# SidRama/Longitudinal-VAE

Hardware: AMD Instinct MI355X
Metric: ELBO-steps/sec (exact-KL L-VAE step, Health-MNIST N=4096 L=16) (higher is better)
Workload: dtype f16x3-split (fp32-equivalent)

## Files before the change

### include/lvae_hip.h

```cpp
#ifndef LVAE_HIP_H
#define LVAE_HIP_H

#include <stddef.h>
#include <stdint.h>

#ifdef __cplusplus
extern "C" {
#endif

#define LVAE_MAX_COMP 16
#define LVAE_MAX_FAC 4
#define LVAE_ERR_LAUNCH (-1000)

enum lvae_factor_kind {
  LVAE_CAT = 0,
  LVAE_BIN = 1,
  LVAE_RBF = 2,
  LVAE_PER = 3,
  LVAE_LIN = 4
};

typedef struct lvae_kernel_spec {
  int32_t n_comp;
  int32_t n_params;
  int32_t n_fac[LVAE_MAX_COMP];
  int32_t scale_idx[LVAE_MAX_COMP];
  int32_t kind[LVAE_MAX_COMP][LVAE_MAX_FAC];
  int32_t dim[LVAE_MAX_COMP][LVAE_MAX_FAC];
  int32_t param_idx[LVAE_MAX_COMP][LVAE_MAX_FAC];
} lvae_kernel_spec;

typedef struct lvae_xview {
  const double* ptr;
  int64_t stride_b;
  int64_t stride_l;
  int64_t ld;
} lvae_xview;


int lvae_gram_f64(const lvae_kernel_spec* spec, lvae_xview x1, lvae_xview x2, int nb, int L, int n1,
                  int n2, const double* params, const double* diag, double* out, int64_t ostride_b,
                  int64_t ostride_l, int64_t ldo, void* stream);
int lvae_gram_f32(const lvae_kernel_spec* spec, lvae_xview x1, lvae_xview x2, int nb, int L, int n1,
                  int n2, const double* params, const double* diag, float* out, int64_t ostride_b,
                  int64_t ostride_l, int64_t ldo, void* stream);

size_t lvae_gram_bwd_workspace_size(int nb, int L, int n1, int n2);
int lvae_gram_bwd_f64(const lvae_kernel_spec* spec, lvae_xview x1, lvae_xview x2, int nb, int L, int n1,
                      int n2, const double* params, const double* G, int64_t gstride_b,
                      int64_t gstride_l, int64_t ldg, double* dparams, double* ddiag, void* workspace,
                      void* stream);

size_t lvae_gram_bwd_x2_workspace_size(int nb, int L, int n1, int n2, int Q);
int lvae_gram_bwd_x2_f64(const lvae_kernel_spec* spec, lvae_xview x1, lvae_xview x2, int nb, int L, int n1, int n2,
                         int Q, const double* params, const double* G, int64_t gstride_b, int64_t gstride_l,
                         int64_t gstride_i, int64_t gstride_j, double* dx2, void* workspace, void* stream);

size_t lvae_gram_matvec_workspace_size(int n1, int n2, int L);
int lvae_gram_matvec_f64(const lvae_kernel_spec* spec, const double* x1, int64_t ld1, int n1, const double* x2,
                         int64_t ld2, int n2, int L, const double* params, const double* diag, const double* v,
                         int64_t ld_v, double* out, int64_t ld_out, void* workspace, void* stream);

int lvae_kl_closed_padded_n(int n);
size_t lvae_kl_closed_workspace_size(int n, int L);


int lvae_kl_closed_fwd_f32(const lvae_kernel_spec* spec, const double* x, int ldx, int n, int L,
                           const double* params, const double* noise, const double* mu, const double* logv,
                           int ld_mu, double* kl, int32_t* info, void* workspace, int need_bwd,
                           void* stream);
int lvae_kl_closed_factor_f32(const lvae_kernel_spec* spec, const double* x, int ldx, int n, int L,
                              const double* params, const double* noise, int32_t* info, void* workspace,
                              void* stream);
int lvae_kl_closed_reduce_f32(const lvae_kernel_spec* spec, const double* x, int ldx, int n, int L,
                              const double* params, const double* noise, const double* mu, const double* logv,
                              int ld_mu, double* kl, void* workspace, int need_bwd, void* stream);

int lvae_kl_closed_bwd_f32(const lvae_kernel_spec* spec, const double* x, int ldx, int n, int L,
                           const double* params, const double* mu, const double* logv, int ld_mu,
                           const double* gkl, double* dmu, double* dlogv, double* dparams, double* dnoise,
                           void* workspace, void* stream);
int lvae_kl_closed_bwd_latent_f32(int n, int L, const double* logv, int ld_mu, const double* gkl, double* dmu,
                                  double* dlogv, void* workspace, void* stream);
int lvae_kl_closed_bwd_hyper_f32(const lvae_kernel_spec* spec, const double* x, int ldx, int n, int L,
                                 const double* params, const double* gkl, double* dparams, double* dnoise,
                                 void* workspace, void* stream);

int lvae_kl_closed_refine_state(int n, int L, const void* workspace, double* est, int32_t* flag, void* stream);

int lvae_kl_closed_hyper_state(int n, int L, const void* workspace, int32_t* on, void* stream);

int lvae_kl_closed_resid_state(int n, int L, const void* workspace, int32_t* covflag, int32_t* binned,
                               void* stream);

size_t lvae_spd_inv_chol_scratch_size(int np_, int L);
int lvae_spd_inv_chol_f32(int np_, int L, float* A, void* scratch, float* Ainv, double* logdet, int32_t* info,
                          void* stream);

int lvae_potrf_f64(int n, int L, const double* A, int64_t lda, int64_t stride_a, double* Lout, int64_t ldo,
                   int64_t stride_o, double* logdet, int32_t* info, void* stream);
size_t lvae_potrf_f32_workspace_size(int n, int L);
int lvae_potrf_f32(int n, int L, const float* A, int64_t lda, int64_t stride_a, float* Lout, int64_t ldo,
                   int64_t stride_o, double* logdet, int32_t* info, void* workspace, void* stream);
size_t lvae_trsm_workspace_size(int n, int L);
int lvae_trsm_f64(int trans, int n, int nrhs, int L, const double* Lf, int64_t ldl, int64_t stride_l, double* B,
                  int64_t ldb, int64_t stride_b, void* workspace, void* stream);
int lvae_trsm_f32(int trans, int n, int nrhs, int L, const float* Lf, int64_t ldl, int64_t stride_l, float* B,
                  int64_t ldb, int64_t stride_b, void* workspace, void* stream);
int lvae_potrs_f64(int n, int nrhs, int L, const double* Lf, int64_t ldl, int64_t stride_l, double* B, int64_t ldb,
                   int64_t stride_b, void* workspace, void* stream);
int lvae_potrs_f32(int n, int nrhs, int L, const float* Lf, int64_t ldl, int64_t stride_l, float* B, int64_t ldb,
                   int64_t stride_b, void* workspace, void* stream);


int lvae_spd_inv_small_f64(int n, int batch, const double* A, int64_t stride, double* Ainv,
                           int64_t stride_out, double* logdet, int32_t* info, void* stream);

int lvae_gemm_small_f64(int ta, int tb, int m, int n, int k, double alpha, const double* A, int lda,
                        int64_t sa1, int64_t sa2, const double* B, int ldb, int64_t sb1, int64_t sb2,
                        double beta, double* C, int ldc, int64_t sc1, int64_t sc2, int nb1, int nb2,
                        void* stream);

typedef struct lvae_hensman_dims {
  int32_t L, M, P_b, T, Q;
  double P_tot;
  double eps;
  int32_t natural_gradient;
  double ng_prior_share;
  const int32_t* seg_len;
  double n_total;
} lvae_hensman_dims;

size_t lvae_hensman_workspace_size(const lvae_hensman_dims* d);
size_t lvae_hensman_iH_offset(const lvae_hensman_dims* d);

int lvae_hensman_fwd_f64(const lvae_kernel_spec* spec0, const lvae_kernel_spec* spec1,
                         const lvae_hensman_dims* d, const double* x, const double* z, const double* m,
                         const double* H, const double* mu, const double* logv, const double* params0,
                         const double* params1, const double* noise, double* kld, double* grad_m,
                         double* grad_H, int32_t* info, void* workspace, void* stream);
int lvae_hensman_fwd_part_f64(int part, const lvae_kernel_spec* spec0, const lvae_kernel_spec* spec1,
                              const lvae_hensman_dims* d, const double* x, const double* z, const double* m,
                              const double* H, const double* mu, const double* logv, const double* params0,
                              const double* params1, const double* noise, double* kld, double* grad_m,
                              double* grad_H, int32_t* info, void* workspace, void* stream);

int lvae_hensman_bwd_f64(const lvae_kernel_spec* spec0, const lvae_kernel_spec* spec1,
                         const lvae_hensman_dims* d, const double* x, const double* z, const double* m,
                         const double* H, const double* mu, const double* logv, const double* params0,
                         const double* params1, const double* noise, const double* gkld, double* dmu,
                         double* dlogv, double* dparams0, double* dparams1, double* dnoise, double* dm,
                         double* dH, void* workspace, void* stream);

size_t lvae_natgrad_workspace_size(int L, int M);
int lvae_natgrad_update_f64(int L, int M, double* m, double* H, const double* grad_m,
                            const double* grad_H, double lr, const double* iH, int32_t* info,
                            void* workspace, void* stream);

typedef struct lvae_dubo_dims {
  int32_t L, M, P, T, Q;
  double eps;
} lvae_dubo_dims;

size_t lvae_dubo_workspace_size(const lvae_dubo_dims* d);

int lvae_dubo_fwd_f64(const lvae_kernel_spec* spec0, const lvae_kernel_spec* spec1, const lvae_dubo_dims* d,
                      const double* x, const double* z, const double* mu, const double* logv,
                      const double* params0, const double* params1, const double* noise, double* dubo,
                      int32_t* info, void* workspace, void* stream);
int lvae_dubo_bwd_f64(const lvae_kernel_spec* spec0, const lvae_kernel_spec* spec1, const lvae_dubo_dims* d,
                      const double* x, const double* z, const double* mu, const double* logv,
                      const double* params0, const double* params1, const double* noise, const double* gdubo,
                      double* dmu, double* dlogv, double* dparams0, double* dparams1, double* dnoise,
                      void* workspace, void* stream);

typedef struct lvae_gp_elbo_dims {
  int32_t L, M, P, T, Q, S;
  double eps;
} lvae_gp_elbo_dims;

size_t lvae_gp_elbo_workspace_size(const lvae_gp_elbo_dims* d);

int lvae_gp_elbo_fwd_f64(const lvae_kernel_spec* spec0, const lvae_kernel_spec* spec1, const lvae_gp_elbo_dims* d,
                         const double* x, const double* z, const double* y, const double* params0,
                         const double* params1, const double* noise, double* elbo, int32_t* info,
                         void* workspace, void* stream);
int lvae_gp_elbo_bwd_f64(const lvae_kernel_spec* spec0, const lvae_kernel_spec* spec1, const lvae_gp_elbo_dims* d,
                         const double* x, const double* z, const double* y, const double* params0,
                         const double* params1, const double* noise, const double* gelbo, double* dy,
                         double* dparams0, double* dparams1, double* dnoise, void* workspace, void* stream);

int lvae_dubo_fwd_seg_f64(const lvae_kernel_spec* spec0, const lvae_kernel_spec* spec1, const lvae_dubo_dims* d,
                          const int32_t* seg_len, const double* x, const double* z, const double* mu,
                          const double* logv, const double* params0, const double* params1, const double* noise,
                          double* dubo, int32_t* info, void* workspace, void* stream);
int lvae_dubo_bwd_seg_f64(const lvae_kernel_spec* spec0, const lvae_kernel_spec* spec1, const lvae_dubo_dims* d,
                          const int32_t* seg_len, const double* x, const double* z, const double* mu,
                          const double* logv, const double* params0, const double* params1, const double* noise,
                          const double* gdubo, double* dmu, double* dlogv, double* dparams0, double* dparams1,
                          double* dnoise, void* workspace, void* stream);
int lvae_gp_elbo_fwd_seg_f64(const lvae_kernel_spec* spec0, const lvae_kernel_spec* spec1,
                             const lvae_gp_elbo_dims* d, const int32_t* seg_len, const double* x, const double* z,
                             const double* y, const double* params0, const double* params1, const double* noise,
                             double* elbo, int32_t* info, void* workspace, void* stream);
int lvae_gp_elbo_bwd_seg_f64(const lvae_kernel_spec* spec0, const lvae_kernel_spec* spec1,
                             const lvae_gp_elbo_dims* d, const int32_t* seg_len, const double* x, const double* z,
                             const double* y, const double* params0, const double* params1, const double* noise,
                             const double* gelbo, double* dy, double* dparams0, double* dparams1, double* dnoise,
                             void* workspace, void* stream);

size_t lvae_bound_dz_workspace_size(int L, int M, int N, int Q);
int lvae_dubo_bwd_z_f64(const lvae_kernel_spec* spec0, const lvae_dubo_dims* d, const double* x, const double* z,
                        const double* params0, double* dz, void* workspace, void* zworkspace, void* stream);
int lvae_gp_elbo_bwd_z_f64(const lvae_kernel_spec* spec0, const lvae_gp_elbo_dims* d, const double* x,
                           const double* z, const double* params0, double* dz, void* workspace, void* zworkspace,
                           void* stream);
int lvae_hensman_bwd_z_f64(const lvae_kernel_spec* spec0, const lvae_hensman_dims* d, const double* x,
                           const double* z, const double* params0, double* dz, void* workspace, void* zworkspace,
                           void* stream);

int lvae_relu_maxpool2_fwd_f32(const float* x, int64_t planes, int H, int W, float* y, uint8_t* idx,
                               void* stream);
int lvae_relu_maxpool2_bwd_f32(const float* gy, const float* y, const uint8_t* idx, int64_t planes, int H,
                               int W, float* gx, void* stream);
size_t lvae_relu_maxpool2_bias_workspace_size(int N, int C);
int lvae_relu_maxpool2_bias_fwd_f32(const float* x, const float* bias, int N, int C, int H, int W, float* y,
                                    uint8_t* idx, void* stream);
int lvae_relu_maxpool2_bias_bwd_f32(const float* gy, const float* y, const uint8_t* idx, int N, int C, int H, int W,
                                    float* gx, float* db, void* workspace, void* stream);
int lvae_conv1_relu_maxpool2_fwd_f32(const float* x, const float* w, const float* bias, int N, int C, int H, int W,
                                     float* y, uint8_t* idx, void* stream);
int lvae_conv3x3_relu_maxpool2_fwd_f32(const float* x, const float* w, const float* bias, int N, int Cin, int C, int H,
                                       int W, float* y, uint8_t* idx, void* stream);
size_t lvae_conv3x3_pool_wgrad_workspace_size(int N, int C, int Cin);
int lvae_conv3x3_pool_wgrad_f32(const float* gy, const float* y, const uint8_t* idx, const float* x, int N, int C,
                                int Cin, int H, int W, float* dw, float* db, void* workspace, void* stream);
size_t lvae_conv3x3_pool_dgrad_lds(int C, int H, int W);
int lvae_conv3x3_pool_dgrad_f32(const float* gy, const float* y, const uint8_t* idx, const float* w, int N, int C,
                                int Cin, int H, int W, float* gx, void* stream);
size_t lvae_deconv2_sigmoid_workspace_size(int N, int Cin, int Hi, int Wi);
int lvae_deconv2_sigmoid_fwd_f32(const float* z, const float* w, const float* bias, int N, int Cin, int Hi, int Wi,
                                 float* out, void* stream);
int lvae_deconv2_sigmoid_bwd_f32(const float* g, const float* out, const float* z, const float* w, int N, int Cin,
                                 int Hi, int Wi, float* gz, float* dw, float* db, void* workspace, void* stream);
int lvae_deconv4s2_relu_fwd_f32(const float* x, const float* w, const float* bias, int N, int Cin, int Cout, int Hi,
                                int Wi, float* y, void* stream);
size_t lvae_deconv4s2_relu_bwd_workspace_size(int N, int Cin, int Cout);
int lvae_deconv4s2_relu_bwd_f32(const float* gy, const float* y, const float* x, const float* w, int N, int Cin,
                                int Cout, int Hi, int Wi, float* dx, float* dw, float* db, void* workspace,
                                void* stream);

size_t lvae_predict_workspace_size(int L, int M, int P, int T, int Nt);
int lvae_predict_f64(const lvae_kernel_spec* spec0, const lvae_kernel_spec* spec1, int L, int M, int Q, int P,
                     int T, const int32_t* seg_len, const int32_t* include, const double* x,
                     const double* mu, const double* z, int Nt, const double* test_x,
                     const double* params0, const double* params1, const double* noise, double eps,
                     double* out, int32_t* info, void* workspace, void* stream);

size_t lvae_predict_exact_workspace_size(int n, int nt, int L);
int lvae_predict_exact_f64(const lvae_kernel_spec* spec, const double* x, int64_t ldx, int n, int L,
                           const double* params, const double* noise, const double* mu, int64_t ld_mu,
                           const double* tx, int64_t ldt, int nt, double* out, int64_t ld_out, int32_t* info,
                           void* workspace, void* stream);

size_t lvae_predict_exact_var_workspace_size(int n, int nt, int L, int chunk);
int lvae_predict_exact_var_f64(const lvae_kernel_spec* spec, const double* x, int64_t ldx, int n, int L,
                               const double* params, const double* noise, const double* mu, int64_t ld_mu,
                               const double* tx, int64_t ldt, int nt, double* out_mean, int64_t ld_out,
                               double* out_var, int64_t ld_var, int add_noise, int chunk, int32_t* info,
                               void* workspace, void* stream);

size_t lvae_predict_var_workspace_size(int L, int M, int P, int T, int Nt);
int lvae_predict_var_f64(const lvae_kernel_spec* spec0, const lvae_kernel_spec* spec1, int L, int M, int Q, int P,
                         int T, const int32_t* seg_len, const int32_t* include, const double* x, const double* mu,
                         const double* z, int Nt, const double* test_x, int n_groups, const int32_t* group_subject,
                         const int32_t* group_start, const double* params0, const double* params1,
                         const double* noise, double eps, double* out, double* out_var, int add_noise, int32_t* info,
                         void* workspace, void* stream);

int lvae_set_early_stream(void* stream);

enum lvae_phase {
  LVAE_PH_GRAM = 0, LVAE_PH_POTRF = 1 , LVAE_PH_POTRI = 2 , LVAE_PH_KL_REDUCE = 3, LVAE_PH_SYRK = 4,
  LVAE_PH_GRAM_BWD = 5, LVAE_PH_BWD_ELEM = 6, LVAE_PH_HENSMAN_FWD = 7, LVAE_PH_HENSMAN_BWD = 8,
  LVAE_PH_NATGRAD = 9, LVAE_PH_SWEEP_UPD = 10 ,
  LVAE_PH_HB_SLAB = 11 , LVAE_N_PHASES = 12
};
int lvae_prof_enable(int on);
int lvae_prof_collect(double* ms, int32_t* count, int n_phases);

const char* lvae_version(void);

int lvae_vae_loss_fwd_f32(const float* recon, const float* x, const float* mask, const float* log_vy, int B, int d,
                          float* mse, float* nll, float* msum, void* stream);
size_t lvae_vae_loss_bwd_partials(int B);
int lvae_vae_loss_bwd_f32(const float* recon, const float* x, const float* mask, const float* log_vy, const float* msum,
                          const float* g_mse, int64_t g_mse_stride, const float* g_nll, int64_t g_nll_stride, int B,
                          int d, float* d_recon, float* dlv_part, void* stream);
int lvae_reparam_fwd_f32(const float* mu, const float* log_var, const float* eps, int64_t n, float* z, void* stream);
int lvae_reparam_bwd_f32(const float* gz, const float* log_var, const float* eps, int64_t n, float* g_log_var,
                         void* stream);
int lvae_param_pack_fwd_f64(int n_raw, int L, int P, const int* cols, const double* const* raws,
                            const double* const* mlogs, double* out, void* stream);
int lvae_bias_relu_fwd_f32(float* y, const float* bias, int N, int C, int HW, void* stream);
size_t lvae_act_bwd_workspace_size(int N, int C);
int lvae_act_bwd_f32(const float* gy, const float* y, int N, int C, int HW, int relu, float* g, float* db,
                     void* workspace, void* stream);
int lvae_step_terms_fwd(const float* mse, const float* nll, int B, const double* kld, float c, double ks, double w,
                        int use_nll, float* rec, float* nl, double* net, double* kd, void* stream);
int lvae_step_terms_bwd(const double* g_net, const float* g_rec, const float* g_nl, const double* g_kd, float c,
                        double ks, double w, int use_nll, float* g_mse, float* g_nll, double* g_kld, void* stream);
int lvae_param_pack_bwd_f64(int n_raw, int L, int P, const int* cols, const double* const* raws,
                            const double* const* mlogs, const double* g, int64_t g_stride0, int64_t g_stride1,
                            double* grad, void* stream);

#ifdef __cplusplus
}
#endif
#endif
```

### longitudinal-vae_amd/csrc/chol_inv.hip

```cpp
#include "prof.hpp"
#include "pv_lds.hpp"
#include "side_stream.hpp"
#include "x3_c16.hpp"

#ifndef LVAE_CI_C16
#define LVAE_CI_C16 1
#endif
#ifndef LVAE_PV_BTRI
#define LVAE_PV_BTRI 1
#endif
#ifndef LVAE_PV_SAMEAB
#define LVAE_PV_SAMEAB 1
#endif
#ifndef LVAE_CI_KREV
#define LVAE_CI_KREV 1
#endif

namespace lvae {

constexpr bool kCiC16 = LVAE_CI_C16 != 0;

#ifndef LVAE_CI_PIPE_MAX_L
#define LVAE_CI_PIPE_MAX_L 2
#endif
// ... 1397 lines not shown
      const int64_t oc = c16_off(l, np_, i * kSwB, j * kSwB);
      c16_tile_planes_out(acc, [&](int) { return -inv * sy; }, g.oh + oc, g.ol + oc);
    } else {
      ci_planes_out(acc, -inv, sy, g.oh + ot, g.ol + ot, np_);
    }
    ci_transposed_out(acc, -inv, lds, [&](int c, int r0, f32x4 v) {
      const int64_t o = kCiC16 ? c16_off(l, np_, j * kSwB + c, i * kSwB + r0) : ott + (int64_t)c * np_ + r0;
      ci_split4(v, sy, g.oth + o, g.otl + o);
    });
    if (threadIdx.x == 0) S.ysc[sl + (int64_t)i * nt + j] = sy;
  } else {
    if constexpr (MODE == kCiLauumKL) {
#pragma unroll
      for (int a = 0; a < 4; ++a)
#pragma unroll
        for (int b = 0; b < 2; ++b) acc[a][b] *= inv;
    }
    const float osc = MODE == kCiLauumKL ? 1.f : inv;
    float* O = g.Kinv + l * np2 + (int64_t)i * kSwB * np_ + (int64_t)j * kSwB;
    float* Ot = g.Kinv + l * np2 + (int64_t)j * kSwB * np_ + (int64_t)i * kSwB;
    const __amdgpu_buffer_rsrc_t ro = __builtin_amdgcn_make_buffer_rsrc(O, (short)0, 0x7fffffff, 0x00020000);
    const int lane = threadIdx.x & 63, w = threadIdx.x >> 6;
    const int vo = (((w >> 2) * 128 + 4 * (lane >> 5)) * np_ + (w & 3) * 64 + (lane & 31)) * 4;
    if (!g.pre) {
#pragma unroll
      for (int a = 0; a < 4; ++a)
#pragma unroll
        for (int e = 0; e < 16; ++e)
#pragma unroll
          for (int b = 0; b < 2; ++b)
            __builtin_amdgcn_raw_buffer_store_b32(__float_as_uint(acc[a][b][e] * osc), ro, vo,
                                                  ((32 * a + (e & 3) + 8 * (e >> 2)) * np_ + 32 * b) * 4, 0);
    }
    if constexpr (MODE == kCiLauumKL) {
      ci_kl_partials(acc, 1.f, g, l, i, j, kl_mu, kl_part);
      const int64_t tb = l * np2 + (int64_t)i * kSwB * np_ + (int64_t)j * kSwB;
      const int64_t tbt = l * np2 + (int64_t)j * kSwB * np_ + (int64_t)i * kSwB;
      const bool hbm = g.bh_out && g.hbon && *g.hbon;
      _Float16* const bho = hbm ? nullptr : g.bh_out;
      _Float16* const blo = hbm ? nullptr : g.bl_out;
      const float sb = bho ? g.bsc[l] : 0.f;
      if (bho && kCiBC16) {
        const int64_t tc = c16_off(l, np_, i * kSwB, j * kSwB);
        c16_tile_planes_out(acc, [&](int b) { return sb * kl_sv[kSwB + sx_col(b)]; }, bho + tc, blo + tc);
      } else if (bho) {
        const __amdgpu_buffer_rsrc_t rh = __builtin_amdgcn_make_buffer_rsrc(bho + tb, (short)0, 0x7fffffff, 0x00020000);
        const __amdgpu_buffer_rsrc_t rl = __builtin_amdgcn_make_buffer_rsrc(blo + tb, (short)0, 0x7fffffff, 0x00020000);
        const int lane = threadIdx.x & 63, w = threadIdx.x >> 6;
        const int vb = (((w >> 2) * 128 + 4 * (lane >> 5)) * np_ + (w & 3) * 64 + (lane & 31)) * 2;
#pragma unroll
        for (int b = 0; b < 2; ++b) {
          const float mc = sb * kl_sv[kSwB + sx_col(b)];
#pragma unroll
          for (int a = 0; a < 4; ++a)
#pragma unroll
            for (int e = 0; e < 16; ++e) {
              const float y = acc[a][b][e] * mc;
              const _Float16 yh = (_Float16)y;
              const _Float16 yl = (_Float16)(y - (float)yh);
              const int so = ((32 * a + (e & 3) + 8 * (e >> 2)) * np_ + 32 * b) * 2;
              __builtin_amdgcn_raw_buffer_store_b16(__builtin_bit_cast(unsigned short, yh), rh, vb, so, 0);
              __builtin_amdgcn_raw_buffer_store_b16(__builtin_bit_cast(unsigned short, yl), rl, vb, so, 0);
            }
        }
      }
      if (i != j && (bho || hbm || LVAE_KL_MIRROR))
        ci_transposed_out(acc, 1.f, lds, [&](int c, int r0, f32x4 v) {
          if (hbm || LVAE_KL_MIRROR) *reinterpret_cast<f32x4*>(Ot + (int64_t)c * np_ + r0) = v;
          if (bho) {
            const f32x4 s4 = *reinterpret_cast<const f32x4*>(&kl_sv[r0]);
            const int64_t o = kCiBC16 ? c16_off(l, np_, j * kSwB + c, i * kSwB + r0) : tbt + (int64_t)c * np_ + r0;
            ci_split4(v * s4, sb, bho + o, blo + o);
          }
        });
    } else if (i != j) {
      ci_transposed_out(acc, inv, lds, [&](int c, int r0, f32x4 v) {
        *reinterpret_cast<f32x4*>(Ot + (int64_t)c * np_ + r0) = v;
      });
    }
  }
}


#define CI_GEMM_LDS                                                                     \
  __shared__ __attribute__((aligned(16))) _Float16 lds[2 * 4 * kSxPart];                \
  __shared__ float sprod[64];                                                           \
  __shared__ uint32_t red;                                                              \
  __shared__ float kl_mu[2 * kSwB], kl_sv[2 * kSwB], kl_part[6 * kSwB];

template <int MODE>
__global__ __launch_bounds__(512) void ci_gemm_kernel(CiGemmArgs g, CiScratch S) {
  CI_GEMM_LDS
  ci_gemm_body<MODE>(g, S, blockIdx.x + g.bid0, lds, sprod, &red, kl_mu, kl_sv, kl_part);
}

template <int M1, int M2>
__global__ __launch_bounds__(512) void ci_pair_kernel(CiGemmArgs g1, CiGemmArgs g2, CiScratch S, int n1) {
  CI_GEMM_LDS
  if ((int)blockIdx.x < n1)
    ci_gemm_body<M1>(g1, S, blockIdx.x, lds, sprod, &red, kl_mu, kl_sv, kl_part);
  else
    ci_gemm_body<M2>(g2, S, blockIdx.x - n1, lds, sprod, &red, kl_mu, kl_sv, kl_part);
}

size_t ci_scratch_bytes(int np_, int L) { return CiScratch(nullptr, np_, L).bytes; }
int ci_factor_f32(int np_, int L, float* A, void* scratch, _Float16* YT, float* Kinv, double* logdet,
                  int32_t* info, hipStream_t st, float* lout = nullptr);

int ci_factor_f32(int np_, int L, float* A, void* scratch, _Float16* YT, float* Kinv, double* logdet,
                  int32_t* info, hipStream_t st, float* lout) {
  if (np_ <= 0 || np_ % kSwB || np_ / kSwB > 64) return -1;
  if (L <= 0) return -2;
  CiScratch S((char*)scratch, np_, L);
  S.lout = lout;
  const int nt = S.nt;
  const int64_t full = (int64_t)L * np_ * np_;
  _Float16* YTh = YT;
  _Float16* YTl = YT + full;
  _Float16* XTh = reinterpret_cast<_Float16*>(Kinv);
  _Float16* XTl = XTh + full;
  _Float16* Yh = XTh;
  _Float16* Yl = XTl;
  auto ok = [](hipError_t e) { return e == hipSuccess; };
  bool pipe = false;
  static const bool early_env = !getenv("LVAE_CI_TRTRI_EARLY") || atoi(getenv("LVAE_CI_TRTRI_EARLY")) != 0;
  static const int free_env = getenv("LVAE_CI_EARLY_FREE") ? atoi(getenv("LVAE_CI_EARLY_FREE")) : -1;
  bool early = false;
  int s_top = 1, ecap = 0;
  while (2 * s_top < nt) s_top *= 2;
  SideStream* sd = nullptr;
  auto trtri_level = [&](int h, int i0, int ni, bool do_x, bool do_y, hipStream_t q, int cap) {
    const int per = ni * h * h, nwg = per * L;
    if (nwg <= 0) return;
    if (do_x) {
      CiGemmArgs gx{S.Lh, S.Ll, YTh, YTl, nullptr, nullptr, XTh, XTl, nullptr, np_, nt, h, per, nwg, i0};
      for (int b0 = 0; b0 < nwg; b0 += cap > 0 ? cap : nwg) {
        gx.bid0 = b0;
        ci_gemm_kernel<kCiX><<<min(nwg - b0, cap > 0 ? cap : nwg), 512, 0, q>>>(gx, S);
      }
    }
    if (do_y) {
      CiGemmArgs gy{Yh, Yl, XTh, XTl, Yh, Yl, YTh, YTl, nullptr, np_, nt, h, per, nwg, i0};
      for (int b0 = 0; b0 < nwg; b0 += cap > 0 ? cap : nwg) {
        gy.bid0 = b0;
        ci_gemm_kernel<kCiY><<<min(nwg - b0, cap > 0 ? cap : nwg), 512, 0, q>>>(gy, S);
      }
    }
  };
  {
    ProfScope ps(LVAE_PH_POTRF, st);
    std::lock_guard<std::recursive_mutex> lock(side_mutex());
    LVAE_TRY(side_stream(sd));
    (void)zero_async(logdet, sizeof(double) * L, st);
    (void)zero_async(info, sizeof(int32_t) * L, st);
    (void)zero_async(S.cnt, CiScratch::cnt_bytes(L, nt), st);
    if (!ok(hipEventRecord(sd->fork, st)) || !ok(hipStreamWaitEvent(sd->s, sd->fork, 0))) return LVAE_ERR_LAUNCH;
    const bool fuse = L <= kCiFuseMaxL;
    const int pmode = lout ? 0 : ci_pipe_mode(np_, L);
    static const bool split_env = !getenv("LVAE_PIVOT_SPLIT") || atoi(getenv("LVAE_PIVOT_SPLIT")) != 0;
    const bool split = split_env;
    static const bool pair = getenv("LVAE_CI_PAIR") && atoi(getenv("LVAE_CI_PAIR")) != 0;
    static const bool la = getenv("LVAE_CI_LOOKAHEAD") && atoi(getenv("LVAE_CI_LOOKAHEAD")) != 0;
    const bool u128 = getenv("LVAE_CI_U128") && atoi(getenv("LVAE_CI_U128")) != 0;
    const bool uring = getenv("LVAE_CI_URING") && atoi(getenv("LVAE_CI_URING")) != 0;
    pipe = pmode > 0;
    hipStreamCaptureStatus cap_st = hipStreamCaptureStatusNone;
    if (!ok(hipStreamIsCapturing(st, &cap_st))) return LVAE_ERR_LAUNCH;
    early = early_env && fuse && !pipe && !lout && nt >= 2 && sd->early && sd->early != st &&
            cap_st == hipStreamCaptureStatusNone;
    {
      const int pvwg = split ? kCiPvG * ((L + 7) / 8 * 8) : L;
      ecap = max(sd->cus - (free_env >= 0 ? free_env : pvwg), max(sd->cus / 4, 1));
    }
    if (fuse) {
      ci_pivot_kernel<1><<<L, 1024, 0, sd->s>>>(A, np_, 0, S, logdet, info, 0, L, g_pivot_prof);
      if (!ok(hipEventRecord(sd->piv[0], sd->s))) return LVAE_ERR_LAUNCH;
      if (nt > 1) ci_prep0_kernel<<<dim3(nt - 1, L), 256, 0, st>>>(A, np_, S);
      if (!ok(hipEventRecord(sd->c, st))) return LVAE_ERR_LAUNCH;
      for (int m = 0; m < nt; ++m) {
        if (m + 1 < nt) {
          if (!ok(hipStreamWaitEvent(sd->s, m == 0 ? sd->c : sd->u2p[(m - 1) & 1], 0))) return LVAE_ERR_LAUNCH;
          if (split) {
            const int Lr = (L + 7) / 8 * 8;
            ci_pivot_kernel<kCiPvG><<<kCiPvG * Lr, 1024, 0, sd->s>>>(A, np_, m + 1, S, logdet, info, 1, L, g_pivot_prof);
          } else {
            ci_pivot_kernel<1><<<L, 1024, 0, sd->s>>>(A, np_, m + 1, S, logdet, info, 1, L, g_pivot_prof);
          }
          if (!ok(hipEventRecord(sd->piv[(m + 1) & 1], sd->s))) return LVAE_ERR_LAUNCH;
        }
        if (!ok(hipStreamWaitEvent(st, sd->piv[m & 1], 0))) return LVAE_ERR_LAUNCH;
        if (pipe && pair) {
          ProfScope pt(LVAE_PH_POTRI, st);
          const int npn = nt - m - 1, ny = m + 16;
          CiGemmArgs gp{nullptr, nullptr, nullptr, nullptr, nullptr, nullptr, nullptr, nullptr, nullptr, np_, nt, m,
                        max(npn, 1), npn * L, 0};
          CiGemmArgs gy{nullptr, nullptr, nullptr, nullptr, nullptr, nullptr, YTh, YTl, nullptr, np_, nt, m, ny, ny * L, 0};
          ci_pair_kernel<kCiPanel, kCiTrY><<<(npn + ny) * L, 512, 0, st>>>(gp, gy, S, npn * L);
          const int n1 = max(nt - m - 2, 0), n2 = max(nt - m - 2, 0) * max(nt - m - 1, 0) / 2, nu = n1 + n2;
          const int perx = (nt - m - 1) * (m + 1), perl = pmode == 2 ? (m + 1) * (m + 2) / 2 : 0;
          CiGemmArgs gu{nullptr, nullptr, nullptr, nullptr, nullptr, nullptr, nullptr, nullptr, A, np_, nt, m,
                        max(nu, 1), nu * L, n1};
          CiGemmArgs gx{S.Lh, S.Ll, YTh, YTl, nullptr, nullptr, nullptr, nullptr, Kinv, np_, nt, m, max(perx + perl, 1),
                        (perx + perl) * L, perx};
          if (nu + perx + perl > 0) ci_pair_kernel<kCiU12c, kCiTrX><<<(nu + perx + perl) * L, 512, 0, st>>>(gu, gx, S, nu * L);
          if (m + 1 < nt && !ok(hipEventRecord(sd->u2p[m & 1], st))) return LVAE_ERR_LAUNCH;
          continue;
        }
        if (m + 1 < nt) {
          ci_panel_kernel<<<dim3(nt - m - 1, L), 512, 0, st>>>(S, np_, m);
          if (early && m == s_top - 1) {
            if (!ok(hipEventRecord(sd->efork, st)) || !ok(hipStreamWaitEvent(sd->early, sd->efork, 0)))
              return LVAE_ERR_LAUNCH;
            {
              ProfScope pe(LVAE_PH_POTRI, sd->early);
              ci_diag_copy_kernel<<<dim3(16 * s_top, L), 256, 0, sd->early>>>(S, np_, Yh, Yl, YTh, YTl, 0);
              for (int h = 1; h < s_top; h *= 2) trtri_level(h, 0, s_top / (2 * h), true, true, sd->early, ecap);
              trtri_level(s_top, 0, 1, true, false, sd->early, ecap);
            }
            if (!ok(hipEventRecord(sd->edone, sd->early))) return LVAE_ERR_LAUNCH;
          }
          const int n1 = nt - m - 2, n2 = (nt - m - 2) * (nt - m - 1) / 2;
          if (n2 > 0 && la && n2 > 1) {
            ProfScope pu(LVAE_PH_SWEEP_UPD, st);
            ci_update_kernel<kCiU12><<<(n1 + 1) * L, 512, 0, st>>>(A, S, np_, m, 1, L, n1, 0);
            if (!ok(hipEventRecord(sd->u2p[m & 1], st))) return LVAE_ERR_LAUNCH;
            ci_update_kernel<kCiU12><<<(n2 - 1) * L, 512, 0, st>>>(A, S, np_, m, n2 - 1, (n2 - 1) * L, 0, 1);
          } else {
            if (n2 > 0) {
              ProfScope pu(LVAE_PH_SWEEP_UPD, st);
              if (u128) {
                ci_update128_kernel<<<4 * (n1 + n2) * L, 256, 0, st>>>(A, S, np_, m, n2, 4 * (n1 + n2) * L, n1);
                ci_prep0_kernel<<<dim3(n1, L), 256, 0, st>>>(A, np_, S, m + 1);
              } else if (uring) {
                ci_update_ring_kernel<kCiU12><<<(n1 + n2) * L, 512, 0, st>>>(A, S, np_, m, n2, n2 * L, n1);
              } else {
                ci_update_kernel<kCiU12><<<(n1 + n2) * L, 512, 0, st>>>(A, S, np_, m, n2, n2 * L, n1);
              }
            }
            if (!ok(hipEventRecord(sd->u2p[m & 1], st))) return LVAE_ERR_LAUNCH;
          }
        }
        if (pipe) {
          ProfScope pt(LVAE_PH_POTRI, st);
          const int pery = m + 16;
          CiGemmArgs gy{nullptr, nullptr, nullptr, nullptr, nullptr, nullptr, YTh, YTl, nullptr, np_, nt, m, pery,
                        pery * L, 0};
          ci_gemm_kernel<kCiTrY><<<pery * L, 512, 0, st>>>(gy, S);
          const int perx = (nt - m - 1) * (m + 1), perl = pmode == 2 ? (m + 1) * (m + 2) / 2 : 0;
          if (perx + perl > 0) {
            CiGemmArgs gx{S.Lh, S.Ll, YTh, YTl, nullptr, nullptr, nullptr, nullptr, Kinv, np_, nt, m, perx + perl,
                          (perx + perl) * L, perx};
            ci_gemm_kernel<kCiTrX><<<(perx + perl) * L, 512, 0, st>>>(gx, S);
          }
        }
      }
    } else {
      if (nt > 1) ci_prep0_kernel<<<dim3(nt - 1, L), 256, 0, sd->s>>>(A, np_, S);
      ci_pivot_kernel<1><<<L, 1024, 0, sd->s>>>(A, np_, 0, S, logdet, info, 0, L, g_pivot_prof);
      if (nt > 1) ci_panel_kernel<<<dim3(nt - 1, L), 512, 0, sd->s>>>(S, np_, 0);
      if (!ok(hipEventRecord(sd->prep, sd->s))) return LVAE_ERR_LAUNCH;
      for (int k = 0; k + 1 < nt; ++k) {
        if (!ok(hipStreamWaitEvent(st, sd->prep, 0))) return LVAE_ERR_LAUNCH;
        const int n1 = nt - k - 1;
        ci_update_kernel<kCiU1><<<n1 * L, 512, 0, st>>>(A, S, np_, k, n1, n1 * L);
        if (!ok(hipEventRecord(sd->c, st))) return LVAE_ERR_LAUNCH;
        if (!ok(hipStreamWaitEvent(sd->s, sd->c, 0))) return LVAE_ERR_LAUNCH;
        ci_pivot_kernel<1><<<L, 1024, 0, sd->s>>>(A, np_, k + 1, S, logdet, info, 0, L, g_pivot_prof);
        if (k + 2 < nt) ci_panel_kernel<<<dim3(nt - k - 2, L), 512, 0, sd->s>>>(S, np_, k + 1);
        if (!ok(hipEventRecord(sd->prep, sd->s))) return LVAE_ERR_LAUNCH;
        const int n2 = (nt - k - 2) * (nt - k - 1) / 2;
        if (n2 > 0) {
          ProfScope pu(LVAE_PH_SWEEP_UPD, st);
          if (u128)
            ci_update128_kernel<<<4 * n2 * L, 256, 0, st>>>(A, S, np_, k, n2, 4 * n2 * L);
          else
            ci_update_kernel<kCiU2><<<n2 * L, 512, 0, st>>>(A, S, np_, k, n2, n2 * L);
        }
      }
      if (!ok(hipStreamWaitEvent(st, sd->prep, 0))) return LVAE_ERR_LAUNCH;
    }
  }
  LVAE_CHECK_LAUNCH();
  if (lout) return 0;
  if (!pipe) {
    ProfScope ps(LVAE_PH_POTRI, st);
    if (early) {
      std::lock_guard<std::recursive_mutex> lock(side_mutex());
      ci_diag_copy_kernel<<<dim3(16 * (nt - s_top), L), 256, 0, st>>>(S, np_, Yh, Yl, YTh, YTl, s_top);
      for (int h = 1; h < s_top; h *= 2) {
        const int i0 = s_top / (2 * h);
        trtri_level(h, i0, (nt + 2 * h - 1) / (2 * h) - i0, true, true, st, 0);
      }
      if (!ok(hipStreamWaitEvent(st, sd->edone, 0))) return LVAE_ERR_LAUNCH;
      trtri_level(s_top, 0, 1, false, true, st, 0);
    } else {
      ci_diag_copy_kernel<<<dim3(16 * nt, L), 256, 0, st>>>(S, np_, Yh, Yl, YTh, YTl, 0);
      for (int h = 1; h < nt; h *= 2) trtri_level(h, 0, (nt + 2 * h - 1) / (2 * h), true, true, st, 0);
    }
  }
  LVAE_CHECK_LAUNCH();
  return 0;
}

__global__ __launch_bounds__(64) void ci_bscale_kernel(CiScratch S, const float* __restrict__ sv, int np_,
                                                       float* __restrict__ bsc) {
  const int l = blockIdx.x, t = threadIdx.x, nt = S.nt;
  const float* ys = S.ysc + (int64_t)l * nt * nt;
  float d = 0.f;
  for (int J = t; J < nt; J += 64) {
    float c = 0.f;
    for (int I = J; I < nt; ++I) {
      const float m = 16384.f / ys[I * nt + J];
      c += 256.f * m * m;
    }
    d = fmaxf(d, c);
  }
  float v = 0.f;
  for (int i = t; i < np_; i += 64) v = fmaxf(v, sv[(int64_t)l * np_ + i]);
#pragma unroll
  for (int o = 32; o > 0; o >>= 1) {
    d = fmaxf(d, __shfl_xor(d, o, 64));
    v = fmaxf(v, __shfl_xor(v, o, 64));
  }
  if (t == 0) bsc[l] = x3_scale(d * v);
}

int ci_lauum_f32(int np_, int L, void* scratch, const _Float16* YT, float* Kinv, const double* mu, const float* sv,
                 float* apart, _Float16* Bh, float* bsc, hipStream_t st, const int* hbon) {
  if (np_ <= 0 || np_ % kSwB || np_ / kSwB > 64) return -1;
  CiScratch S((char*)scratch, np_, L);
  const int nt = S.nt, per = nt * (nt + 1) / 2, nwg = per * L;
  const int64_t full = (int64_t)L * np_ * np_;
  ProfScope ps(LVAE_PH_POTRI, st);
  CiGemmArgs gl{YT, YT + full, YT, YT + full, nullptr, nullptr, nullptr, nullptr, Kinv, np_, nt, 0, per, nwg, 0};
  gl.pre = ci_pipe_mode(np_, L) == 2;
  if (mu) {
    gl.mu = mu;
    gl.sv = sv;
    gl.apart = apart;
    gl.bh_out = Bh;
    gl.bl_out = Bh ? Bh + full : nullptr;
    gl.bsc = bsc;
    gl.hbon = hbon;
    if (Bh) ci_bscale_kernel<<<L, 64, 0, st>>>(S, sv, np_, bsc);
    ci_gemm_kernel<kCiLauumKL><<<nwg, 512, 0, st>>>(gl, S);
  } else {
    ci_gemm_kernel<kCiLauum><<<nwg, 512, 0, st>>>(gl, S);
  }
  LVAE_CHECK_LAUNCH();
  return 0;
}

int ci_lauum_flagged_f32(int np_, int L, void* scratch, const _Float16* YT, float* Kinv, const int* flag, hipStream_t st) {
  if (np_ <= 0 || np_ % kSwB || np_ / kSwB > 64) return -1;
  CiScratch S((char*)scratch, np_, L);
  const int nt = S.nt, per = nt * (nt + 1) / 2, nwg = per * L;
  const int64_t full = (int64_t)L * np_ * np_;
  CiGemmArgs gl{YT, YT + full, YT, YT + full, nullptr, nullptr, nullptr, nullptr, Kinv, np_, nt, 0, per, nwg, 0};
  gl.dimflag = flag;
  ci_gemm_kernel<kCiLauum><<<nwg, 512, 0, st>>>(gl, S);
  LVAE_CHECK_LAUNCH();
  return 0;
}

int ci_pipe_mode_of(int np_, int L) { return ci_pipe_mode(np_, L); }

const float* ci_ysc_ptr(void* scratch, int np_, int L) { return CiScratch((char*)scratch, np_, L).ysc; }

int ci_potrf_f32(int np_, int L, float* A, void* scratch, double* logdet, int32_t* info, hipStream_t st) {
  return ci_factor_f32(np_, L, A, scratch, nullptr, nullptr, logdet, info, st, A);
}

int ci_inverse_f32(int np_, int L, float* A, void* scratch, _Float16* YT, float* Kinv, double* logdet,
                   int32_t* info, hipStream_t st) {
  LVAE_TRY(ci_factor_f32(np_, L, A, scratch, YT, Kinv, logdet, info, st));
  return ci_lauum_f32(np_, L, scratch, YT, Kinv, nullptr, nullptr, nullptr, nullptr, nullptr, st, nullptr);
}

}

extern "C" {
void lvae_dev_pivot_prof(void* buf) { lvae::g_pivot_prof = (unsigned long long*)buf; }
size_t lvae_spd_inv_chol_scratch_size(int np_, int L) {
  return lvae::ci_scratch_bytes(np_, L) + lvae::align256((size_t)L * np_ * np_ * 2 * sizeof(_Float16));
}
int lvae_spd_inv_chol_f32(int np_, int L, float* A, void* scratch, float* Ainv, double* logdet, int32_t* info,
                          void* stream) {
  if (!A) return -3;
  if (!scratch || ((uintptr_t)scratch & 255)) return -4;
  if (!Ainv) return -5;
  if (!logdet) return -6;
  if (!info) return -7;
  if (np_ <= 0 || np_ % lvae::kSwB || np_ / lvae::kSwB > 64) return -1;
  if (L <= 0) return -2;
  char* yt = (char*)scratch + lvae::ci_scratch_bytes(np_, L);
  return lvae::ci_inverse_f32(np_, L, A, scratch, (_Float16*)yt, Ainv, logdet, info, (hipStream_t)stream);
}
}
```

### longitudinal-vae_amd/csrc/kl_closed.hip

```cpp
#include "common.hpp"
#include "side_stream.hpp"
#include "prof.hpp"
#include "x3_c16.hpp"

#include <unordered_set>


#ifndef LVAE_ALPHA_WG
#define LVAE_ALPHA_WG 4096
#endif

namespace lvae {

int kl_gram_fill(const lvae_kernel_spec* spec, const double* x, int ldx, int n, int np_, int L,
                 const double* params, const double* noise, float* K, int* covflag, hipStream_t st);
size_t kl_gram_bwd_partials_bytes(int np_, int L);
int kl_gram_bwd(const lvae_kernel_spec* spec, const double* x, int ldx, int n, int np_, int L,
                const double* params, const float* Kinv, const float* S, const float* Sx, int nsplit,
                const double* alpha, const double* kdiag, const float* v, const double* gkl, double* part,
                double* dparams, double* dnoise, const int* covflag, void* hbws, const int* hbon, hipStream_t st);
int syrk_x3_splits(int np_, int L);
int syrk_tiles_f32(int np_, int L, const float* bsc, const _Float16* planes, float* S, float* Sx, hipStream_t st,
                   const int* skip);
size_t kl_hyper_bytes(int np_, int L);
struct HbDev;
HbDev* kl_hyper_dev(void* base, int np_, int L);
int kl_hyper_plan(const lvae_kernel_spec* spec, const double* x, int ldx, int n, int np_, int L, void* wsbase,
                  const int* covflag, hipStream_t st);
int ci_factor_f32(int np_, int L, float* A, void* scratch, _Float16* YT, float* Kinv, double* logdet,
                  int32_t* info, hipStream_t st, float* lout = nullptr);
int ci_lauum_f32(int np_, int L, void* scratch, const _Float16* YT, float* Kinv, const double* mu, const float* sv,
                 float* apart, _Float16* Bh, float* bsc, hipStream_t st, const int* hbon);
size_t ci_scratch_bytes(int np_, int L);
size_t kl_resid_partials_bytes(int np_, int L);
int kl_gram_resid(const lvae_kernel_spec* spec, const double* x, int ldx, int n, int np_, int L,
                  const double* params, const double* noise, const double* alpha0, const double* muc, double* part,
                  double* res, void* rbws, hipStream_t st);
size_t kl_resid_bins_bytes(int np_, int L, int ncomp);
bool kl_resid_bins_enabled(const lvae_kernel_spec* spec, int n);
int kl_resid_bins_plan(const lvae_kernel_spec* spec, const double* x, int ldx, int n, int np_, int L, void* wsbuf,
                       hipStream_t st);
int* kl_resid_bins_okflag(void* wsbuf);
size_t kl_refine_bytes(int np_, int L);
int kl_refine_gate(const lvae_kernel_spec* spec, const double* x, int ldx, int n, int np_, int L, const double* params,
                   const double* noise, const double* kdiag, double* est, int* flag, hipStream_t st);
int kl_refine_apply(const lvae_kernel_spec* spec, const double* x, int ldx, int n, int np_, int L, const double* params,
                    const double* noise, const float* Kinv, double* kdiag, double* K64, double* part, const int* flag,
                    hipStream_t st);
int ci_lauum_flagged_f32(int np_, int L, void* scratch, const _Float16* YT, float* Kinv, const int* flag, hipStream_t st);
const float* ci_ysc_ptr(void* scratch, int np_, int L);
int ci_pipe_mode_of(int np_, int L);
size_t kl_refine_part_bytes(int np_, int L);
int kl_refine_diag(const lvae_kernel_spec* spec, const double* x, int ldx, int n, int np_, int L,
                   const double* params, const double* noise, const float* Kinv, double* kdiag, double* K64,
                   double* part, double* est, int* flag, hipStream_t st);

struct KLWorkspace {
  float *A, *Kinv, *v, *sv;
  float* Sx;
  _Float16* planes;
  _Float16* Bp;
  float* bsc;
  float* apart;
  char* chol;
  double *mu, *alpha, *res, *kdiag, *logdet, *part, *rpart;
  int* covflag;
  char* rb;
  double* K64;
  char* hb;
  const int* hbon;
  double* rest;
  int* rflag;
  double* ypart;
  double* yvec;
  double* K64e;
  size_t bytes, bytes_base;
  KLWorkspace(char* base, int np_, int L) {
    size_t off = 0;
    auto take = [&](size_t b) {
      char* p = base ? base + off : nullptr;
      off += align256(b);
      return p;
    };
    const size_t mat = (size_t)L * np_ * np_ * sizeof(float);
    A = (float*)take(mat);
    Bp = reinterpret_cast<_Float16*>(A);
    Kinv = (float*)take(mat);
    planes = (_Float16*)take(mat);
    K64 = reinterpret_cast<double*>(planes);
    take(kl_refine_bytes(np_, L) - mat);
    v = (float*)take((size_t)L * np_ * sizeof(float));
    sv = (float*)take((size_t)L * np_ * sizeof(float));
    bsc = (float*)take((size_t)L * sizeof(float));
    apart = (float*)take((size_t)L * (np_ / 256) * np_ * sizeof(float));
    mu = (double*)take((size_t)L * np_ * sizeof(double));
    alpha = (double*)take((size_t)L * np_ * sizeof(double));
    res = (double*)take((size_t)L * np_ * sizeof(double));
    kdiag = (double*)take((size_t)L * np_ * sizeof(double));
    logdet = (double*)take((size_t)L * sizeof(double));
    chol = take(ci_scratch_bytes(np_, L));
    part = (double*)take(kl_gram_bwd_partials_bytes(np_, L));
    rpart = (double*)take(kl_resid_partials_bytes(np_, L));
    covflag = (int*)take(sizeof(int));
    rb = take(kl_resid_bins_bytes(np_, L, LVAE_MAX_COMP));
    Sx = (float*)take(mat * (size_t)(syrk_x3_splits(np_, L) - 1));
    hb = take(kl_hyper_bytes(np_, L));
    hbon = base ? reinterpret_cast<const int*>(kl_hyper_dev(hb, np_, L)) : nullptr;
    rest = (double*)take((size_t)L * sizeof(double));
    rflag = (int*)take((size_t)L * sizeof(int));
    bytes_base = off;
    ypart = (double*)take(2 * (size_t)L * (np_ / 256) * np_ * sizeof(double));
    yvec = (double*)take((size_t)L * np_ * sizeof(double));
    K64e = (double*)take(kl_refine_bytes(np_, L));
    bytes = off;
  }
};

__global__ void kl_prep_kernel(const double* __restrict__ mu, const double* __restrict__ logv, int ld, int n, int np_,
                               int L, double* __restrict__ muc, float* __restrict__ v, float* __restrict__ sv) {
  const int i = blockIdx.x * blockDim.x + threadIdx.x, l = blockIdx.y;
  if (i >= np_) return;
  const bool in = i < n;
  muc[(int64_t)l * np_ + i] = in ? mu[(int64_t)i * ld + l] : 0.0;
  const double vv = in ? exp(logv[(int64_t)i * ld + l]) : 0.0;
  v[(int64_t)l * np_ + i] = (float)vv;
  sv[(int64_t)l * np_ + i] = (float)sqrt(vv);
}

__global__ __launch_bounds__(256) void kl_alpha0_kernel(const float* __restrict__ apart, const float* __restrict__ Kinv,
                                                        int np_, double* __restrict__ alpha,
                                                        double* __restrict__ kdiag) {
  const int l = blockIdx.y, nt = np_ / 256;
  const int p = blockIdx.x * 256 + threadIdx.x;
  const float* ap = apart + (int64_t)l * nt * np_ + p;
  double s = 0.0;
  for (int q = 0; q < nt; ++q) s += (double)ap[(int64_t)q * np_];
  const int64_t o = (int64_t)l * np_ + p;
  alpha[o] = s;
  kdiag[o] = (double)Kinv[(int64_t)l * np_ * np_ + (int64_t)p * np_ + p];
}

__global__ __launch_bounds__(256) void kl_alpha_kernel(const float* __restrict__ Kinv, const double* __restrict__ u,
                                                       int np_, const double* base, double* alpha) {
  const int l = blockIdx.y, lane = threadIdx.x & 63;
  const int i = blockIdx.x * 4 + (threadIdx.x >> 6);
  if (i >= np_) return;
  const float* row = Kinv + (int64_t)l * np_ * np_ + (int64_t)i * np_;
  const double* m = u + (int64_t)l * np_;
  double acc = 0.0;
  for (int j = lane * 4; j < np_; j += 256) {
    const float4 k4 = *reinterpret_cast<const float4*>(row + j);
    acc += (double)k4.x * m[j] + (double)k4.y * m[j + 1] + (double)k4.z * m[j + 2] + (double)k4.w * m[j + 3];
  }
  acc = wave_sum(acc);
  if (lane == 0) {
    const int64_t o = (int64_t)l * np_ + i;
    alpha[o] = base[o] + acc;
  }
}

__device__ inline void alpha_tri_index(int t, int& I, int& J) {
  int r = (int)((sqrt(8.0 * (double)t + 1.0) - 1.0) * 0.5);
  while ((r + 1) * (r + 2) / 2 <= t) ++r;
  while (r * (r + 1) / 2 > t) --r;
  I = r;
  J = t - r * (r + 1) / 2;
}
__global__ __launch_bounds__(256) void kl_alpha_sym_kernel(const float* __restrict__ Kinv,
                                                           const double* __restrict__ u, int np_,
                                                           double* __restrict__ part, int ntiles) {
  __shared__ double cred[4][64];
  const int G = gridDim.x, l = blockIdx.y, tid = threadIdx.x, tr = tid >> 4, tc = tid & 15, wv = tid >> 6;
  const int nt = np_ / 64;
  const float* K = Kinv + (int64_t)l * np_ * np_;
  const double* ul = u + (int64_t)l * np_;
  for (int t = blockIdx.x; t < ntiles; t += G) {
    int I, J;
    alpha_tri_index(t, I, J);
    const int i0 = I * 64, j0 = J * 64;
    float4 k[4];
#pragma unroll
    for (int a = 0; a < 4; ++a)
      k[a] = *reinterpret_cast<const float4*>(K + (int64_t)(i0 + 4 * tr + a) * np_ + j0 + 4 * tc);
    double uj[4], ui[4];
#pragma unroll
    for (int c = 0; c < 4; ++c) uj[c] = ul[j0 + 4 * tc + c];
#pragma unroll
    for (int a = 0; a < 4; ++a) ui[a] = ul[i0 + 4 * tr + a];
    double rs[4], cs[4];
#pragma unroll
    for (int a = 0; a < 4; ++a) {
      rs[a] = (double)k[a].x * uj[0] + (double)k[a].y * uj[1] + (double)k[a].z * uj[2] + (double)k[a].w * uj[3];
#pragma unroll
      for (int o = 1; o < 16; o <<= 1) rs[a] += __shfl_xor(rs[a], o, 64);
    }
    if (tc == 0) {
      double* pr = part + ((int64_t)l * nt + J) * np_ + i0 + 4 * tr;
#pragma unroll
      for (int a = 0; a < 4; ++a) pr[a] = rs[a];
    }
    if (I != J) {
      cs[0] = (double)k[0].x * ui[0] + (double)k[1].x * ui[1] + (double)k[2].x * ui[2] + (double)k[3].x * ui[3];
      cs[1] = (double)k[0].y * ui[0] + (double)k[1].y * ui[1] + (double)k[2].y * ui[2] + (double)k[3].y * ui[3];
      cs[2] = (double)k[0].z * ui[0] + (double)k[1].z * ui[1] + (double)k[2].z * ui[2] + (double)k[3].z * ui[3];
      cs[3] = (double)k[0].w * ui[0] + (double)k[1].w * ui[1] + (double)k[2].w * ui[2] + (double)k[3].w * ui[3];
#pragma unroll
      for (int c = 0; c < 4; ++c) {
        cs[c] += __shfl_xor(cs[c], 16, 64);
        cs[c] += __shfl_xor(cs[c], 32, 64);
      }
      __syncthreads();
      if ((tid & 63) < 16) {
#pragma unroll
        for (int c = 0; c < 4; ++c) cred[wv][4 * tc + c] = cs[c];
      }
      __syncthreads();
      if (tid < 64)
        part[((int64_t)l * nt + I) * np_ + j0 + tid] = ((cred[0][tid] + cred[1][tid]) + cred[2][tid]) + cred[3][tid];
    }
  }
}

__global__ __launch_bounds__(256) void kl_alpha_reduce(const double* __restrict__ part, const double* base, int np_,
                                                       double* alpha) {
  const int i = blockIdx.x * 256 + threadIdx.x, l = blockIdx.y, nt = np_ / 64;
  if (i >= np_) return;
  double acc = 0.0;
  const double* pl = part + (int64_t)l * nt * np_ + i;
  for (int s = 0; s < nt; s += 4) {
    const double v0 = pl[(int64_t)s * np_], v1 = pl[(int64_t)(s + 1) * np_];
    const double v2 = pl[(int64_t)(s + 2) * np_], v3 = pl[(int64_t)(s + 3) * np_];
    acc += v0;
    acc += v1;
    acc += v2;
    acc += v3;
  }
  const int64_t o = (int64_t)l * np_ + i;
  alpha[o] = base[o] + acc;
}

template <bool UPPER, bool SUMSQ>
__global__ __launch_bounds__(256) void kl_ymv_kernel(const _Float16* __restrict__ hi, const _Float16* __restrict__ lo,
                                                     const float* __restrict__ ysc, int np_, const double* __restrict__ x,
                                                     double* __restrict__ part, double* __restrict__ part2) {
  __shared__ double xs[256];
  const int l = blockIdx.y, tid = threadIdx.x, nt = np_ / 256;
  int R, C;
  alpha_tri_index(blockIdx.x, R, C);
  if (UPPER) {
    const int t = R;
    R = C;
    C = t;
  }
  xs[tid] = x[(int64_t)l * np_ + C * 256 + tid];
  const float s = ysc[((int64_t)l * nt + max(R, C)) * nt + min(R, C)];
  __syncthreads();
  const int row = R * 256 + tid;
  const bool sw = (tid >> 3) & 1;
  const int64_t base = (int64_t)l * np_ * np_ + ((int64_t)R * (np_ >> 4) + C * 16) * kC16Part + tid * 16;
  const uint4* ph = reinterpret_cast<const uint4*>(hi + base);
  const uint4* pl = reinterpret_cast<const uint4*>(lo + base);
  constexpr int kChunkU4 = kC16Part / 8;
  double acc = 0.0, sq = 0.0;
#pragma unroll 4
  for (int c = 0; c < 16; ++c) {
    const uint4 h0 = ph[c * kChunkU4], h1 = ph[c * kChunkU4 + 1];
    const uint4 l0 = pl[c * kChunkU4], l1 = pl[c * kChunkU4 + 1];
    _Float16 hv[16], lv[16];
    *reinterpret_cast<uint4*>(hv) = sw ? h1 : h0;
    *reinterpret_cast<uint4*>(hv + 8) = sw ? h0 : h1;
    *reinterpret_cast<uint4*>(lv) = sw ? l1 : l0;
    *reinterpret_cast<uint4*>(lv + 8) = sw ? l0 : l1;
#pragma unroll
    for (int kk = 0; kk < 16; ++kk) {
      const double v = (double)((float)hv[kk] + (float)lv[kk]);
      acc += v * xs[c * 16 + kk];
      if (SUMSQ) sq += v * v;
    }
  }
  const double inv = 1.0 / (double)s;
  part[((int64_t)l * nt + C) * np_ + row] = acc * inv;
  if (SUMSQ) part2[((int64_t)l * nt + C) * np_ + row] = sq * inv * inv;
}

template <bool UPPER>
__global__ __launch_bounds__(256) void kl_ymv_reduce(const double* __restrict__ part, const double* base, int np_,
                                                     double* out) {
  const int i = blockIdx.x * 256 + threadIdx.x, l = blockIdx.y, nt = np_ / 256, R = blockIdx.x;
  const double* p = part + (int64_t)l * nt * np_ + i;
  double acc = 0.0;
  for (int C = UPPER ? R : 0; C <= (UPPER ? nt - 1 : R); ++C) acc += p[(int64_t)C * np_];
  const int64_t o = (int64_t)l * np_ + i;
  out[o] = (base ? base[o] : 0.0) + acc;
}

__global__ __launch_bounds__(256) void kl_finalize_kernel(const double* __restrict__ muc, const double* __restrict__ logv,
                                                          int ld, const double* __restrict__ alpha,
                                                          const double* __restrict__ kdiag,
                                                          const double* __restrict__ logdet, int n, int np_,
                                                          double* __restrict__ kl) {
  __shared__ double red[4];
  const int l = blockIdx.x, tid = threadIdx.x;
  double quad = 0.0, tr = 0.0, slv = 0.0;
  for (int i = tid; i < n; i += 256) {
    const double lv = logv[(int64_t)i * ld + l];
    quad += muc[(int64_t)l * np_ + i] * alpha[(int64_t)l * np_ + i];
    tr += exp(lv) * kdiag[(int64_t)l * np_ + i];
    slv += lv;
  }
  quad = block_sum<256>(quad, red);
  tr = block_sum<256>(tr, red);
  slv = block_sum<256>(slv, red);
  if (tid == 0) kl[l] = 0.5 * (tr + quad - (double)n + logdet[l] - slv);
}

__global__ void kl_bwd_elem_kernel(const double* __restrict__ logv, int ld, int n, int np_, int L,
                                   const double* __restrict__ alpha, const double* __restrict__ kdiag,
                                   const double* __restrict__ gkl, double* __restrict__ dmu,
                                   double* __restrict__ dlogv) {
  const int64_t e = (int64_t)blockIdx.x * blockDim.x + threadIdx.x;
  if (e >= (int64_t)n * L) return;
  const int i = (int)(e / L), l = (int)(e % L);
  const double g = gkl[l];
  dmu[(int64_t)i * ld + l] = g * alpha[(int64_t)l * np_ + i];
  dlogv[(int64_t)i * ld + l] = 0.5 * g * (exp(logv[(int64_t)i * ld + l]) * kdiag[(int64_t)l * np_ + i] - 1.0);
}

}

using namespace lvae;

extern "C" {

int lvae_kl_closed_padded_n(int n) { return ((n + 255) / 256) * 256; }

static bool kl_early_env() {
  const char* e = getenv("LVAE_KL_EARLY");
  return e && atoi(e) != 0;
}

static std::unordered_set<const void*>& kl_early_set() {
  static std::unordered_set<const void*> s;
  return s;
}
static void kl_early_record(const void* workspace, bool early) {
  std::lock_guard<std::recursive_mutex> lock(side_mutex());
  if (early) kl_early_set().insert(workspace);
  else kl_early_set().erase(workspace);
}
static bool kl_early(const void* workspace) {
  std::lock_guard<std::recursive_mutex> lock(side_mutex());
  return kl_early_set().count(workspace) != 0;
}

constexpr int kKlMaxN = 64 * 256;
static int kl_check_problem(const lvae_kernel_spec* spec, const double* x, int ldx, int n, int L,
                            const double* params) {
  if (!spec || spec->n_comp < 1 || spec->n_comp > LVAE_MAX_COMP) return -1;
  int qmin = 1;
  for (int r = 0; r < spec->n_comp; ++r) {
    if (spec->n_fac[r] < 0 || spec->n_fac[r] > LVAE_MAX_FAC) return -1;
    for (int f = 0; f < spec->n_fac[r]; ++f) {
      if (spec->dim[r][f] < 0) return -1;
      qmin = spec->dim[r][f] + 1 > qmin ? spec->dim[r][f] + 1 : qmin;
    }
  }
  if (!x) return -2;
  if (ldx < qmin) return -3;
  if (n <= 0 || n > kKlMaxN) return -4;
  if (L <= 0) return -5;
  if (!params) return -6;
  return 0;
}
static bool kl_bad_ws(const void* workspace) { return !workspace || ((uintptr_t)workspace & 255); }

size_t kl_hyper_offset_in_kl_ws(int np_, int L) {
  char* const fake = reinterpret_cast<char*>(uintptr_t(1) << 20);
  KLWorkspace ws(fake, np_, L);
  return (size_t)(ws.hb - fake);
}

size_t lvae_kl_closed_workspace_size(int n, int L) {
  const int np_ = lvae_kl_closed_padded_n(n);
  if (n <= 0 || n > kKlMaxN || L <= 0) return 0;
  const KLWorkspace ws(nullptr, np_, L);
  return kl_early_env() ? ws.bytes : ws.bytes_base;
}

int lvae_kl_closed_factor_f32(const lvae_kernel_spec* spec, const double* x, int ldx, int n, int L,
                              const double* params, const double* noise, int32_t* info, void* workspace,
                              void* stream) {
  LVAE_TRY(kl_check_problem(spec, x, ldx, n, L, params));
  if (!noise) return -7;
  if (!info) return -8;
  if (kl_bad_ws(workspace)) return -9;
  hipStream_t st = (hipStream_t)stream;
  const int np_ = lvae_kl_closed_padded_n(n);
  KLWorkspace ws((char*)workspace, np_, L);
  kl_early_record(workspace, kl_early_env() && ci_pipe_mode_of(np_, L) == 0);
  const bool rb_on = kl_resid_bins_enabled(spec, n);
  std::unique_lock<std::recursive_mutex> lock(side_mutex(), std::defer_lock);
  SideStream* sd = nullptr;
  auto ok = [](hipError_t e) { return e == hipSuccess; };
  if (rb_on) {
    lock.lock();
    LVAE_TRY(side_stream(sd));
  }
  {
    ProfScope ps(LVAE_PH_GRAM, st);
    LVAE_TRY(kl_gram_fill(spec, x, ldx, n, np_, L, params, noise, ws.A, ws.covflag, st));
  }
  if (rb_on && !ok(hipEventRecord(sd->rbx, st))) return LVAE_ERR_LAUNCH;
  if (!rb_on) {
    LVAE_TRY(kl_hyper_plan(spec, x, ldx, n, np_, L, ws.hb, ws.covflag, st));
    LVAE_TRY(zero_async(kl_resid_bins_okflag(ws.rb), sizeof(int), st));
  }
  LVAE_TRY(ci_factor_f32(np_, L, ws.A, ws.chol, ws.planes, ws.Kinv, ws.logdet, info, st));
  if (rb_on) {
    if (!ok(hipStreamWaitEvent(sd->s, sd->rbx, 0))) return LVAE_ERR_LAUNCH;
    LVAE_TRY(kl_resid_bins_plan(spec, x, ldx, n, np_, L, ws.rb, sd->s));
    LVAE_TRY(kl_hyper_plan(spec, x, ldx, n, np_, L, ws.hb, ws.covflag, sd->s));
    if (!ok(hipEventRecord(sd->rb, sd->s))) return LVAE_ERR_LAUNCH;
    if (!ok(hipStreamWaitEvent(st, sd->rb, 0))) return LVAE_ERR_LAUNCH;
  }
  LVAE_CHECK_LAUNCH();
  return 0;
}


static void kl_ymv(const KLWorkspace& ws, const float* ysc, int np_, int L, bool upper, const double* x,
                   const double* base, double* out, double* sumsq, hipStream_t st) {
  const int nt = np_ / 256, ntri = nt * (nt + 1) / 2;
  const int64_t full = (int64_t)L * np_ * np_;
  double* p2 = ws.ypart + (int64_t)L * nt * np_;
  if (!upper) {
    const _Float16* yh = reinterpret_cast<const _Float16*>(ws.Kinv);
    kl_ymv_kernel<false, false><<<dim3(ntri, L), 256, 0, st>>>(yh, yh + full, ysc, np_, x, ws.ypart, nullptr);
    kl_ymv_reduce<false><<<dim3(nt, L), 256, 0, st>>>(ws.ypart, base, np_, out);
  } else {
    const _Float16* th = ws.planes;
    if (sumsq) {
      kl_ymv_kernel<true, true><<<dim3(ntri, L), 256, 0, st>>>(th, th + full, ysc, np_, x, ws.ypart, p2);
      kl_ymv_reduce<true><<<dim3(nt, L), 256, 0, st>>>(p2, nullptr, np_, sumsq);
    } else {
      kl_ymv_kernel<true, false><<<dim3(ntri, L), 256, 0, st>>>(th, th + full, ysc, np_, x, ws.ypart, nullptr);
    }
    kl_ymv_reduce<true><<<dim3(nt, L), 256, 0, st>>>(ws.ypart, base, np_, out);
  }
}

int lvae_kl_closed_reduce_f32(const lvae_kernel_spec* spec, const double* x, int ldx, int n, int L,
                              const double* params, const double* noise, const double* mu, const double* logv,
                              int ld_mu, double* kl, void* workspace, int need_bwd, void* stream) {
  LVAE_TRY(kl_check_problem(spec, x, ldx, n, L, params));
  if (!noise) return -7;
  if (!mu) return -8;
  if (!logv) return -9;
  if (ld_mu < L) return -10;
  if (!kl) return -11;
  if (kl_bad_ws(workspace)) return -12;
  hipStream_t st = (hipStream_t)stream;
  const int np_ = lvae_kl_closed_padded_n(n);
  KLWorkspace ws((char*)workspace, np_, L);
  ProfScope ps(LVAE_PH_KL_REDUCE, st);
  kl_prep_kernel<<<dim3(cdiv(np_, 256), L), 256, 0, st>>>(mu, logv, ld_mu, n, np_, L, ws.mu, ws.v, ws.sv);
  const bool rb_on = kl_resid_bins_enabled(spec, n);
  if (kl_early(workspace)) {
    const float* ysc = ci_ysc_ptr(ws.chol, np_, L);
    kl_ymv(ws, ysc, np_, L, false, ws.mu, nullptr, ws.yvec, nullptr, st);
    kl_ymv(ws, ysc, np_, L, true, ws.yvec, nullptr, ws.alpha, ws.kdiag, st);
    LVAE_TRY(kl_gram_resid(spec, x, ldx, n, np_, L, params, noise, ws.alpha, ws.mu, ws.rpart, ws.res,
                           rb_on ? ws.rb : nullptr, st));
    kl_ymv(ws, ysc, np_, L, false, ws.res, nullptr, ws.yvec, nullptr, st);
    kl_ymv(ws, ysc, np_, L, true, ws.yvec, ws.alpha, ws.alpha, nullptr, st);
    LVAE_TRY(kl_refine_gate(spec, x, ldx, n, np_, L, params, noise, ws.kdiag, ws.rest, ws.rflag, st));
    LVAE_TRY(ci_lauum_flagged_f32(np_, L, ws.chol, ws.planes, ws.Kinv, ws.rflag, st));
    LVAE_TRY(kl_refine_apply(spec, x, ldx, n, np_, L, params, noise, ws.Kinv, ws.kdiag, ws.K64e, ws.rpart, ws.rflag,
                             st));
    kl_finalize_kernel<<<L, 256, 0, st>>>(ws.mu, logv, ld_mu, ws.alpha, ws.kdiag, ws.logdet, n, np_, kl);
    LVAE_CHECK_LAUNCH();
    return 0;
  }
  LVAE_TRY(ci_lauum_f32(np_, L, ws.chol, ws.planes, ws.Kinv, ws.mu, ws.sv, ws.apart, need_bwd ? ws.Bp : nullptr,
                        ws.bsc, st, ws.hbon));
  kl_alpha0_kernel<<<dim3(np_ / 256, L), 256, 0, st>>>(ws.apart, ws.Kinv, np_, ws.alpha, ws.kdiag);
  LVAE_TRY(kl_gram_resid(spec, x, ldx, n, np_, L, params, noise, ws.alpha, ws.mu, ws.rpart, ws.res,
                         rb_on ? ws.rb : nullptr, st));
  {
    const int nt64 = np_ / 64, ntiles = nt64 * (nt64 + 1) / 2;
    int G = (LVAE_ALPHA_WG + L - 1) / L;
    G = G < ntiles ? G : ntiles;
    kl_alpha_sym_kernel<<<dim3(G, L), 256, 0, st>>>(ws.Kinv, ws.res, np_, ws.rpart, ntiles);
    kl_alpha_reduce<<<dim3(np_ / 256, L), 256, 0, st>>>(ws.rpart, ws.alpha, np_, ws.alpha);
  }
  LVAE_TRY(kl_refine_diag(spec, x, ldx, n, np_, L, params, noise, ws.Kinv, ws.kdiag, ws.K64, ws.rpart, ws.rest,
                          ws.rflag, st));
  kl_finalize_kernel<<<L, 256, 0, st>>>(ws.mu, logv, ld_mu, ws.alpha, ws.kdiag, ws.logdet, n, np_, kl);
  LVAE_CHECK_LAUNCH();
  return 0;
}

int lvae_kl_closed_fwd_f32(const lvae_kernel_spec* spec, const double* x, int ldx, int n, int L, const double* params,
                           const double* noise, const double* mu, const double* logv, int ld_mu, double* kl,
                           int32_t* info, void* workspace, int need_bwd, void* stream) {
  LVAE_TRY(kl_check_problem(spec, x, ldx, n, L, params));
  if (!noise) return -7;
  if (!mu) return -8;
  if (!logv) return -9;
  if (ld_mu < L) return -10;
  if (!kl) return -11;
  if (!info) return -12;
  if (kl_bad_ws(workspace)) return -13;
  LVAE_TRY(lvae_kl_closed_factor_f32(spec, x, ldx, n, L, params, noise, info, workspace, stream));
  return lvae_kl_closed_reduce_f32(spec, x, ldx, n, L, params, noise, mu, logv, ld_mu, kl, workspace, need_bwd, stream);
}

int lvae_kl_closed_bwd_hyper_f32(const lvae_kernel_spec* spec, const double* x, int ldx, int n, int L,
                                 const double* params, const double* gkl, double* dparams, double* dnoise,
                                 void* workspace, void* stream) {
  LVAE_TRY(kl_check_problem(spec, x, ldx, n, L, params));
  if (!gkl) return -10;
  if (!dparams) return -13;
  if (!dnoise) return -14;
  if (kl_bad_ws(workspace)) return -15;
  hipStream_t st = (hipStream_t)stream;
  const int np_ = lvae_kl_closed_padded_n(n);
  KLWorkspace ws((char*)workspace, np_, L);
  if (kl_early(workspace)) {
    ProfScope ps(LVAE_PH_KL_REDUCE, st);
    LVAE_TRY(ci_lauum_f32(np_, L, ws.chol, ws.planes, ws.Kinv, ws.mu, ws.sv, ws.apart, ws.Bp, ws.bsc, st, ws.hbon));
  }
  float* S = reinterpret_cast<float*>(ws.planes);
  {
    ProfScope ps(LVAE_PH_SYRK, st);
    LVAE_TRY(syrk_tiles_f32(np_, L, ws.bsc, ws.Bp, S, ws.Sx, st, ws.hbon));
  }
  {
    ProfScope ps(LVAE_PH_GRAM_BWD, st);
    LVAE_TRY(kl_gram_bwd(spec, x, ldx, n, np_, L, params, ws.Kinv, S, ws.Sx, syrk_x3_splits(np_, L), ws.alpha,
                         ws.kdiag, ws.v, gkl, ws.part, dparams, dnoise, ws.covflag, ws.hb, ws.hbon, st));
  }
  LVAE_CHECK_LAUNCH();
  return 0;
}

int lvae_kl_closed_bwd_latent_f32(int n, int L, const double* logv, int ld_mu, const double* gkl, double* dmu,
                                  double* dlogv, void* workspace, void* stream) {
  if (n <= 0 || n > kKlMaxN) return -4;
  if (L <= 0) return -5;
  if (!logv) return -8;
  if (ld_mu < L) return -9;
  if (!gkl) return -10;
  if (!dmu) return -11;
  if (!dlogv) return -12;
  if (kl_bad_ws(workspace)) return -15;
  hipStream_t st = (hipStream_t)stream;
  const int np_ = lvae_kl_closed_padded_n(n);
  KLWorkspace ws((char*)workspace, np_, L);
  ProfScope ps(LVAE_PH_BWD_ELEM, st);
  const int64_t tot = (int64_t)n * L;
  kl_bwd_elem_kernel<<<cdiv(tot, 256), 256, 0, st>>>(logv, ld_mu, n, np_, L, ws.alpha, ws.kdiag, gkl, dmu, dlogv);
  LVAE_CHECK_LAUNCH();
  return 0;
}

int lvae_kl_closed_bwd_f32(const lvae_kernel_spec* spec, const double* x, int ldx, int n, int L, const double* params,
                           const double* mu, const double* logv, int ld_mu, const double* gkl, double* dmu,
                           double* dlogv, double* dparams, double* dnoise, void* workspace, void* stream) {
  (void)mu;
  LVAE_TRY(kl_check_problem(spec, x, ldx, n, L, params));
  if (!logv) return -8;
  if (ld_mu < L) return -9;
  if (!gkl) return -10;
  if (!dmu) return -11;
  if (!dlogv) return -12;
  if (!dparams) return -13;
  if (!dnoise) return -14;
  if (kl_bad_ws(workspace)) return -15;
  LVAE_TRY(lvae_kl_closed_bwd_latent_f32(n, L, logv, ld_mu, gkl, dmu, dlogv, workspace, stream));
  return lvae_kl_closed_bwd_hyper_f32(spec, x, ldx, n, L, params, gkl, dparams, dnoise, workspace, stream);
}

int lvae_kl_closed_refine_state(int n, int L, const void* workspace, double* est, int32_t* flag, void* stream) {
  if (n <= 0 || n > kKlMaxN) return -1;
  if (L <= 0) return -2;
  if (kl_bad_ws(workspace)) return -3;
  if (!est) return -4;
  if (!flag) return -5;
  const int np_ = lvae_kl_closed_padded_n(n);
  KLWorkspace ws((char*)workspace, np_, L);
  hipStream_t st = (hipStream_t)stream;
  if (copy_words_async(est, ws.rest, (size_t)L * sizeof(double), st) != 0 ||
      copy_words_async(flag, ws.rflag, (size_t)L * sizeof(int32_t), st) != 0)
    return LVAE_ERR_LAUNCH;
  return 0;
}

int lvae_kl_closed_resid_state(int n, int L, const void* workspace, int32_t* covflag, int32_t* binned, void* stream) {
  if (n <= 0 || n > kKlMaxN) return -1;
  if (L <= 0) return -2;
  if (kl_bad_ws(workspace)) return -3;
  if (!covflag) return -4;
  if (!binned) return -5;
  const int np_ = lvae_kl_closed_padded_n(n);
  KLWorkspace ws((char*)workspace, np_, L);
  hipStream_t st = (hipStream_t)stream;
  if (copy_words_async(covflag, ws.covflag, sizeof(int32_t), st) != 0 ||
      copy_words_async(binned, kl_resid_bins_okflag(ws.rb), sizeof(int32_t), st) != 0)
    return LVAE_ERR_LAUNCH;
  return 0;
}

const char* lvae_version(void) { return "lvae_hip 0.1.0 gfx950"; }

}
```

### longitudinal-vae_amd/csrc/side_stream.cpp

```cpp
#include "side_stream.hpp"

#include "lvae_hip.h"

namespace lvae {

namespace {
constexpr int kMaxDev = 64;
SideStream g_side[kMaxDev];
}

std::recursive_mutex& side_mutex() {
  static std::recursive_mutex mu;
  return mu;
}

int side_stream(SideStream*& out) {
  int dev = 0;
  if (hipGetDevice(&dev) != hipSuccess || dev < 0 || dev >= kMaxDev) return LVAE_ERR_LAUNCH;
  SideStream& sd = g_side[dev];
  if (!sd.s) {
    int least = 0, greatest = 0;
    (void)hipDeviceGetStreamPriorityRange(&least, &greatest);
    hipDeviceProp_t prop;
    if (hipGetDeviceProperties(&prop, dev) != hipSuccess) return LVAE_ERR_LAUNCH;
    sd.cus = prop.multiProcessorCount;
    for (hipEvent_t* e : {&sd.fork, &sd.prep, &sd.c, &sd.u2p[0], &sd.u2p[1], &sd.piv[0], &sd.piv[1], &sd.rbx, &sd.rb,
                          &sd.efork, &sd.edone})
      if (!*e && hipEventCreateWithFlags(e, hipEventDisableTiming) != hipSuccess) return LVAE_ERR_LAUNCH;
    if (hipStreamCreateWithPriority(&sd.s, hipStreamNonBlocking, greatest) != hipSuccess) return LVAE_ERR_LAUNCH;
  }
  out = &sd;
  return 0;
}

}

extern "C" int lvae_set_early_stream(void* stream) {
  std::lock_guard<std::recursive_mutex> lock(lvae::side_mutex());
  lvae::SideStream* sd = nullptr;
  if (int rc = lvae::side_stream(sd)) return rc;
  sd->early = (hipStream_t)stream;
  return 0;
}
```

### longitudinal-vae_amd/csrc/side_stream.hpp

```cpp
#pragma once
#include <hip/hip_runtime.h>

#include <mutex>

namespace lvae {

struct SideStream {
  hipStream_t s = nullptr;
  hipEvent_t fork = nullptr, prep = nullptr, c = nullptr, u2p[2] = {}, piv[2] = {};
  hipEvent_t rbx = nullptr, rb = nullptr;
  hipStream_t early = nullptr;
  hipEvent_t efork = nullptr, edone = nullptr;
  int cus = 0;
};

std::recursive_mutex& side_mutex();
int side_stream(SideStream*& out);

}
```

### longitudinal-vae_amd/lvae_amd/_lib.py

```python
import ctypes
import os

import torch

_HERE = os.path.dirname(os.path.abspath(__file__))
LIB_PATH = os.path.join(_HERE, "liblvae_hip.so")

MAX_COMP = 16
MAX_FAC = 4
ERR_LAUNCH = -1000

CAT, BIN, RBF, PER, LIN = 0, 1, 2, 3, 4
KIND_CODE = {"cat": CAT, "bin": BIN, "rbf": RBF, "per": PER, "lin": LIN}
N_FACTOR_PARAMS = {"cat": 0, "bin": 0, "rbf": 1, "per": 2, "lin": 0}


class KernelSpec(ctypes.Structure):
    _fields_ = [
        ("n_comp", ctypes.c_int32),
        ("n_params", ctypes.c_int32),
        ("n_fac", ctypes.c_int32 * MAX_COMP),
        ("scale_idx", ctypes.c_int32 * MAX_COMP),
        ("kind", (ctypes.c_int32 * MAX_FAC) * MAX_COMP),
        ("dim", (ctypes.c_int32 * MAX_FAC) * MAX_COMP),
        ("param_idx", (ctypes.c_int32 * MAX_FAC) * MAX_COMP),
    ]


class XView(ctypes.Structure):
    _fields_ = [("ptr", ctypes.c_void_p), ("stride_b", ctypes.c_int64), ("stride_l", ctypes.c_int64),
                ("ld", ctypes.c_int64)]


class HensmanDims(ctypes.Structure):
    _fields_ = [("L", ctypes.c_int32), ("M", ctypes.c_int32), ("P_b", ctypes.c_int32), ("T", ctypes.c_int32),
                ("Q", ctypes.c_int32), ("P_tot", ctypes.c_double), ("eps", ctypes.c_double),
                ("natural_gradient", ctypes.c_int32), ("ng_prior_share", ctypes.c_double),
                ("seg_len", ctypes.c_void_p), ("n_total", ctypes.c_double)]


class DuboDims(ctypes.Structure):
    _fields_ = [("L", ctypes.c_int32), ("M", ctypes.c_int32), ("P", ctypes.c_int32), ("T", ctypes.c_int32),
                ("Q", ctypes.c_int32), ("eps", ctypes.c_double)]


class GpElboDims(ctypes.Structure):
    _fields_ = [("L", ctypes.c_int32), ("M", ctypes.c_int32), ("P", ctypes.c_int32), ("T", ctypes.c_int32),
                ("Q", ctypes.c_int32), ("S", ctypes.c_int32), ("eps", ctypes.c_double)]


def make_spec(components):
    if len(components) > MAX_COMP:
        raise ValueError(f"at most {MAX_COMP} additive components")
    s = KernelSpec()
    s.n_comp = len(components)
    p = 0
    for r, comp in enumerate(components):
        if not 1 <= len(comp) <= MAX_FAC:
            raise ValueError(f"component {r}: 1..{MAX_FAC} factors")
        s.n_fac[r] = len(comp)
        s.scale_idx[r] = p
        p += 1
        for f, (kind, dim) in enumerate(comp):
            s.kind[r][f] = KIND_CODE[kind]
            s.dim[r][f] = int(dim)
            if N_FACTOR_PARAMS[kind]:
                s.param_idx[r][f] = p
                p += N_FACTOR_PARAMS[kind]
            else:
                s.param_idx[r][f] = -1
    s.n_params = p
    return s


_VP, _I32, _I64, _D, _SZ = ctypes.c_void_p, ctypes.c_int32, ctypes.c_int64, ctypes.c_double, ctypes.c_size_t
_SPEC = ctypes.POINTER(KernelSpec)
_DIMS = ctypes.POINTER(HensmanDims)
_DDIMS = ctypes.POINTER(DuboDims)
_GDIMS = ctypes.POINTER(GpElboDims)

SIGNATURES = {
    "lvae_gram_f64": (_I32, [_SPEC, XView, XView, _I32, _I32, _I32, _I32, _VP, _VP, _VP, _I64, _I64, _I64, _VP]),
    "lvae_gram_f32": (_I32, [_SPEC, XView, XView, _I32, _I32, _I32, _I32, _VP, _VP, _VP, _I64, _I64, _I64, _VP]),
    "lvae_gram_bwd_workspace_size": (_SZ, [_I32, _I32, _I32, _I32]),
    "lvae_gram_bwd_f64": (_I32, [_SPEC, XView, XView, _I32, _I32, _I32, _I32, _VP, _VP, _I64, _I64, _I64, _VP,
                                 _VP, _VP, _VP]),
    "lvae_gram_bwd_x2_workspace_size": (_SZ, [_I32, _I32, _I32, _I32, _I32]),
    "lvae_gram_bwd_x2_f64": (_I32, [_SPEC, XView, XView, _I32, _I32, _I32, _I32, _I32, _VP, _VP, _I64, _I64, _I64,
                                    _I64, _VP, _VP, _VP]),
    "lvae_bound_dz_workspace_size": (_SZ, [_I32, _I32, _I32, _I32]),
    "lvae_dubo_bwd_z_f64": (_I32, [_SPEC, _DDIMS, _VP, _VP, _VP, _VP, _VP, _VP, _VP]),
    "lvae_gp_elbo_bwd_z_f64": (_I32, [_SPEC, _GDIMS, _VP, _VP, _VP, _VP, _VP, _VP, _VP]),
    "lvae_hensman_bwd_z_f64": (_I32, [_SPEC, _DIMS, _VP, _VP, _VP, _VP, _VP, _VP, _VP]),
    "lvae_kl_closed_padded_n": (_I32, [_I32]),
    "lvae_kl_closed_workspace_size": (_SZ, [_I32, _I32]),
    "lvae_kl_closed_factor_f32": (_I32, [_SPEC, _VP, _I32, _I32, _I32, _VP, _VP, _VP, _VP, _VP]),
    "lvae_kl_closed_reduce_f32": (_I32, [_SPEC, _VP, _I32, _I32, _I32, _VP, _VP, _VP, _VP, _I32, _VP, _VP, _I32,
                                         _VP]),
    "lvae_kl_closed_fwd_f32": (_I32, [_SPEC, _VP, _I32, _I32, _I32, _VP, _VP, _VP, _VP, _I32, _VP, _VP, _VP,
                                      _I32, _VP]),
    "lvae_kl_closed_bwd_f32": (_I32, [_SPEC, _VP, _I32, _I32, _I32, _VP, _VP, _VP, _I32, _VP, _VP, _VP, _VP,
                                      _VP, _VP, _VP]),
    "lvae_kl_closed_bwd_latent_f32": (_I32, [_I32, _I32, _VP, _I32, _VP, _VP, _VP, _VP, _VP]),
    "lvae_kl_closed_bwd_hyper_f32": (_I32, [_SPEC, _VP, _I32, _I32, _I32, _VP, _VP, _VP, _VP, _VP, _VP]),
    "lvae_kl_closed_refine_state": (_I32, [_I32, _I32, _VP, _VP, _VP, _VP]),
    "lvae_kl_closed_hyper_state": (_I32, [_I32, _I32, _VP, _VP, _VP]),
    "lvae_kl_closed_resid_state": (_I32, [_I32, _I32, _VP, _VP, _VP, _VP]),
    "lvae_vae_loss_fwd_f32": (_I32, [_VP, _VP, _VP, _VP, _I32, _I32, _VP, _VP, _VP, _VP]),
    "lvae_vae_loss_bwd_partials": (_SZ, [_I32]),
    "lvae_bias_relu_fwd_f32": (_I32, [_VP, _VP, _I32, _I32, _I32, _VP]),
    "lvae_act_bwd_workspace_size": (_SZ, [_I32, _I32]),
    "lvae_act_bwd_f32": (_I32, [_VP, _VP, _I32, _I32, _I32, _I32, _VP, _VP, _VP, _VP]),
    "lvae_vae_loss_bwd_f32": (_I32, [_VP, _VP, _VP, _VP, _VP, _VP, _I64, _VP, _I64, _I32, _I32, _VP, _VP, _VP]),
    "lvae_reparam_fwd_f32": (_I32, [_VP, _VP, _VP, _I64, _VP, _VP]),
    "lvae_reparam_bwd_f32": (_I32, [_VP, _VP, _VP, _I64, _VP, _VP]),
    "lvae_step_terms_fwd": (_I32, [_VP, _VP, _I32, _VP, ctypes.c_float, _D, _D, _I32, _VP, _VP, _VP, _VP, _VP]),
    "lvae_step_terms_bwd": (_I32, [_VP, _VP, _VP, _VP, ctypes.c_float, _D, _D, _I32, _VP, _VP, _VP, _VP]),
    "lvae_param_pack_fwd_f64": (_I32, [_I32, _I32, _I32, _VP, _VP, _VP, _VP, _VP]),
    "lvae_param_pack_bwd_f64": (_I32, [_I32, _I32, _I32, _VP, _VP, _VP, _VP, _I64, _I64, _VP, _VP]),
    "lvae_spd_inv_small_f64": (_I32, [_I32, _I32, _VP, _I64, _VP, _I64, _VP, _VP, _VP]),
    "lvae_gemm_small_f64": (_I32, [_I32, _I32, _I32, _I32, _I32, _D, _VP, _I32, _I64, _I64, _VP, _I32, _I64,
                                   _I64, _D, _VP, _I32, _I64, _I64, _I32, _I32, _VP]),
    "lvae_hensman_workspace_size": (_SZ, [_DIMS]),
    "lvae_hensman_fwd_f64": (_I32, [_SPEC, _SPEC, _DIMS, _VP, _VP, _VP, _VP, _VP, _VP, _VP, _VP, _VP, _VP, _VP,
                                    _VP, _VP, _VP, _VP]),
    "lvae_hensman_fwd_part_f64": (_I32, [_I32, _SPEC, _SPEC, _DIMS, _VP, _VP, _VP, _VP, _VP, _VP, _VP, _VP, _VP, _VP,
                                         _VP, _VP, _VP, _VP, _VP]),
    "lvae_hensman_bwd_f64": (_I32, [_SPEC, _SPEC, _DIMS, _VP, _VP, _VP, _VP, _VP, _VP, _VP, _VP, _VP, _VP, _VP,
                                    _VP, _VP, _VP, _VP, _VP, _VP, _VP, _VP]),
    "lvae_natgrad_workspace_size": (_SZ, [_I32, _I32]),
    "lvae_natgrad_update_f64": (_I32, [_I32, _I32, _VP, _VP, _VP, _VP, _D, _VP, _VP, _VP, _VP]),
    "lvae_hensman_iH_offset": (_SZ, [_DIMS]),
    "lvae_dubo_workspace_size": (_SZ, [_DDIMS]),
    "lvae_dubo_fwd_f64": (_I32, [_SPEC, _SPEC, _DDIMS, _VP, _VP, _VP, _VP, _VP, _VP, _VP, _VP, _VP, _VP, _VP]),
    "lvae_dubo_bwd_f64": (_I32, [_SPEC, _SPEC, _DDIMS, _VP, _VP, _VP, _VP, _VP, _VP, _VP, _VP, _VP, _VP, _VP, _VP,
                                 _VP, _VP, _VP]),
    "lvae_gp_elbo_workspace_size": (_SZ, [_GDIMS]),
    "lvae_gp_elbo_fwd_f64": (_I32, [_SPEC, _SPEC, _GDIMS, _VP, _VP, _VP, _VP, _VP, _VP, _VP, _VP, _VP, _VP]),
    "lvae_gp_elbo_bwd_f64": (_I32, [_SPEC, _SPEC, _GDIMS, _VP, _VP, _VP, _VP, _VP, _VP, _VP, _VP, _VP, _VP, _VP,
                                    _VP, _VP]),
    "lvae_dubo_fwd_seg_f64": (_I32, [_SPEC, _SPEC, _DDIMS, _VP, _VP, _VP, _VP, _VP, _VP, _VP, _VP, _VP, _VP, _VP,
                                     _VP]),
    "lvae_dubo_bwd_seg_f64": (_I32, [_SPEC, _SPEC, _DDIMS, _VP, _VP, _VP, _VP, _VP, _VP, _VP, _VP, _VP, _VP, _VP,
                                     _VP, _VP, _VP, _VP, _VP]),
    "lvae_gp_elbo_fwd_seg_f64": (_I32, [_SPEC, _SPEC, _GDIMS, _VP, _VP, _VP, _VP, _VP, _VP, _VP, _VP, _VP, _VP,
                                        _VP]),
    "lvae_gp_elbo_bwd_seg_f64": (_I32, [_SPEC, _SPEC, _GDIMS, _VP, _VP, _VP, _VP, _VP, _VP, _VP, _VP, _VP, _VP, _VP,
                                        _VP, _VP, _VP]),
    "lvae_relu_maxpool2_fwd_f32": (_I32, [_VP, _I64, _I32, _I32, _VP, _VP, _VP]),
    "lvae_relu_maxpool2_bwd_f32": (_I32, [_VP, _VP, _VP, _I64, _I32, _I32, _VP, _VP]),
    "lvae_relu_maxpool2_bias_workspace_size": (_SZ, [_I32, _I32]),
    "lvae_conv1_relu_maxpool2_fwd_f32": (_I32, [_VP, _VP, _VP, _I32, _I32, _I32, _I32, _VP, _VP, _VP]),
    "lvae_relu_maxpool2_bias_fwd_f32": (_I32, [_VP, _VP, _I32, _I32, _I32, _I32, _VP, _VP, _VP]),
    "lvae_relu_maxpool2_bias_bwd_f32": (_I32, [_VP, _VP, _VP, _I32, _I32, _I32, _I32, _VP, _VP, _VP, _VP]),
    "lvae_conv3x3_pool_wgrad_workspace_size": (_SZ, [_I32, _I32, _I32]),
    "lvae_deconv2_sigmoid_workspace_size": (_SZ, [_I32, _I32, _I32, _I32]),
    "lvae_deconv2_sigmoid_fwd_f32": (_I32, [_VP, _VP, _VP, _I32, _I32, _I32, _I32, _VP, _VP]),
    "lvae_deconv2_sigmoid_bwd_f32": (_I32, [_VP, _VP, _VP, _VP, _I32, _I32, _I32, _I32, _VP, _VP, _VP, _VP, _VP]),
    "lvae_conv3x3_pool_wgrad_f32": (_I32, [_VP, _VP, _VP, _VP, _I32, _I32, _I32, _I32, _I32, _VP, _VP, _VP, _VP]),
    "lvae_conv3x3_relu_maxpool2_fwd_f32": (_I32, [_VP, _VP, _VP, _I32, _I32, _I32, _I32, _I32, _VP, _VP, _VP]),
    "lvae_deconv4s2_relu_fwd_f32": (_I32, [_VP, _VP, _VP, _I32, _I32, _I32, _I32, _I32, _VP, _VP]),
    "lvae_deconv4s2_relu_bwd_workspace_size": (_SZ, [_I32, _I32, _I32]),
    "lvae_deconv4s2_relu_bwd_f32": (_I32, [_VP, _VP, _VP, _VP, _I32, _I32, _I32, _I32, _I32, _VP, _VP, _VP, _VP,
                                            _VP]),
    "lvae_conv3x3_pool_dgrad_lds": (_SZ, [_I32, _I32, _I32]),
    "lvae_conv3x3_pool_dgrad_f32": (_I32, [_VP, _VP, _VP, _VP, _I32, _I32, _I32, _I32, _I32, _VP, _VP]),
    "lvae_spd_inv_chol_scratch_size": (_SZ, [_I32, _I32]),
    "lvae_spd_inv_chol_f32": (_I32, [_I32, _I32, _VP, _VP, _VP, _VP, _VP, _VP]),
    "lvae_potrf_f64": (_I32, [_I32, _I32, _VP, _I64, _I64, _VP, _I64, _I64, _VP, _VP, _VP]),
    "lvae_potrf_f32_workspace_size": (_SZ, [_I32, _I32]),
    "lvae_potrf_f32": (_I32, [_I32, _I32, _VP, _I64, _I64, _VP, _I64, _I64, _VP, _VP, _VP, _VP]),
    "lvae_trsm_workspace_size": (_SZ, [_I32, _I32]),
    "lvae_trsm_f64": (_I32, [_I32, _I32, _I32, _I32, _VP, _I64, _I64, _VP, _I64, _I64, _VP, _VP]),
    "lvae_trsm_f32": (_I32, [_I32, _I32, _I32, _I32, _VP, _I64, _I64, _VP, _I64, _I64, _VP, _VP]),
    "lvae_potrs_f64": (_I32, [_I32, _I32, _I32, _VP, _I64, _I64, _VP, _I64, _I64, _VP, _VP]),
    "lvae_potrs_f32": (_I32, [_I32, _I32, _I32, _VP, _I64, _I64, _VP, _I64, _I64, _VP, _VP]),
    "lvae_predict_workspace_size": (_SZ, [_I32, _I32, _I32, _I32, _I32]),
    "lvae_predict_f64": (_I32, [_SPEC, _SPEC, _I32, _I32, _I32, _I32, _I32, _VP, _VP, _VP, _VP, _VP, _I32, _VP, _VP,
                                _VP, _VP, _D, _VP, _VP, _VP, _VP]),
    "lvae_gram_matvec_workspace_size": (_SZ, [_I32, _I32, _I32]),
    "lvae_gram_matvec_f64": (_I32, [_SPEC, _VP, _I64, _I32, _VP, _I64, _I32, _I32, _VP, _VP, _VP, _I64, _VP, _I64,
                                    _VP, _VP]),
    "lvae_predict_exact_workspace_size": (_SZ, [_I32, _I32, _I32]),
    "lvae_predict_exact_f64": (_I32, [_SPEC, _VP, _I64, _I32, _I32, _VP, _VP, _VP, _I64, _VP, _I64, _I32, _VP, _I64,
                                      _VP, _VP, _VP]),
    "lvae_predict_exact_var_workspace_size": (_SZ, [_I32, _I32, _I32, _I32]),
    "lvae_predict_exact_var_f64": (_I32, [_SPEC, _VP, _I64, _I32, _I32, _VP, _VP, _VP, _I64, _VP, _I64, _I32, _VP,
                                          _I64, _VP, _I64, _I32, _I32, _VP, _VP, _VP]),
    "lvae_predict_var_workspace_size": (_SZ, [_I32, _I32, _I32, _I32, _I32]),
    "lvae_predict_var_f64": (_I32, [_SPEC, _SPEC, _I32, _I32, _I32, _I32, _I32, _VP, _VP, _VP, _VP, _VP, _I32, _VP,
                                    _I32, _VP, _VP, _VP, _VP, _VP, _D, _VP, _VP, _I32, _VP, _VP, _VP]),
    "lvae_prof_enable": (_I32, [_I32]),
    "lvae_set_early_stream": (_I32, [_VP]),
    "lvae_prof_collect": (_I32, [_VP, _VP, _I32]),
    "lvae_version": (ctypes.c_char_p, []),
}

_lib = None


def load(path=LIB_PATH):
    global _lib
    if _lib is not None:
        return _lib
    if path == LIB_PATH:
        path = os.environ.get("LVAE_LIB", path)
    if not os.path.exists(path):
        raise RuntimeError(f"lvae_amd: HIP library {path} not built (run __graft_entry__.build())")
    lib = ctypes.CDLL(path)
    missing = [name for name in SIGNATURES if not hasattr(lib, name)]
    if missing:
        raise RuntimeError(f"lvae_amd: {path} lacks declared symbols {missing} (stale build?)")
    for name, (res, args) in SIGNATURES.items():
        fn = getattr(lib, name)
        fn.restype = res
        fn.argtypes = args
    _lib = lib
    return lib


def lib():
    if not torch.cuda.is_available():
        raise RuntimeError("lvae_amd: no GPU visible; the GP-prior hot path runs only through HIP")
    return load()


def stream_ptr(device=None):
    return ctypes.c_void_p(torch.cuda.current_stream(device).cuda_stream)


def ptr(t):
    if t is None:
        return None
    if not t.is_cuda:
        raise ValueError("lvae_amd: tensor must live on the GPU")
    return ctypes.c_void_p(t.data_ptr())


def check(rc, what):
    if rc != 0:
        if rc == ERR_LAUNCH:
            raise RuntimeError(f"lvae_amd: {what}: HIP launch failed")
        raise ValueError(f"lvae_amd: {what}: bad argument #{-rc}")


def xview(t, stride_b, stride_l):
    assert t.dtype == torch.float64 and t.stride(-1) == 1
    return XView(ctypes.c_void_p(t.data_ptr()), int(stride_b), int(stride_l), int(t.stride(-2)))


PHASES = ["gram", "potrf", "potri", "kl_reduce", "syrk", "gram_bwd", "bwd_elem", "hensman_fwd", "hensman_bwd",
          "natgrad", "sweep_update", "hb_slab"]


def prof_enable(on=True):
    lib().lvae_prof_enable(1 if on else 0)


def prof_collect():
    n = len(PHASES)
    ms = (ctypes.c_double * n)()
    cnt = (ctypes.c_int32 * n)()
    check(lib().lvae_prof_collect(ms, cnt, n), "prof_collect")
    return {PHASES[i]: (ms[i], cnt[i]) for i in range(n)}
```

### longitudinal-vae_amd/lvae_amd/elbo.py

```python
import contextlib
import os

import torch

from . import _lib
from .kernels import kernel_spec_and_params

_SYNC_CHECKS = True
_PENDING = []


def set_sync_checks(on):
    global _SYNC_CHECKS
    _SYNC_CHECKS = bool(on)


def _check_info(info, what):
    if _SYNC_CHECKS:
        bad = info.nonzero()
        if bad.numel():
            l = int(bad[0, 0])
            raise torch.linalg.LinAlgError(
                f"{what}: latent dim {l}: the leading minor of order {int(info[l])} is not positive-definite")
    else:
        _PENDING.append((info, what))


def take_pending():
    global _PENDING
    pend, _PENDING = _PENDING, []
    return pend


def check_pending(pend=None):
    for info, what in (take_pending() if pend is None else pend):
        bad = info.nonzero()
        if bad.numel():
            l = int(bad[0, 0])
            raise torch.linalg.LinAlgError(f"{what}: latent dim {l}: leading minor {int(info[l])} not PD")


_ASYNC_FACTOR = os.environ.get("LVAE_ASYNC_FACTOR", "1") != "0"
_FACTOR_POOL = None


def _factor_pool():
    global _FACTOR_POOL
    if _FACTOR_POOL is None:
        from concurrent.futures import ThreadPoolExecutor
        _FACTOR_POOL = ThreadPoolExecutor(max_workers=1, thread_name_prefix="lvae-factor")
    return _FACTOR_POOL


class KLFactor:

    def __init__(self, spec, params, noise, x, stream):
        lib = _lib.lib()
        self.spec, self.params, self.noise = spec, params, noise
        L = params.shape[0]
        n = x.shape[0]
        dev = params.device
        main = torch.cuda.current_stream(dev)
        stream.wait_stream(main)
        with torch.cuda.stream(stream):
            self.x64 = x.detach().to(torch.float64).contiguous()
            self.p = params.detach().to(torch.float64).contiguous()
            self.nz = noise.detach().to(torch.float64).reshape(L).contiguous()
            self.ws = torch.empty(int(lib.lvae_kl_closed_workspace_size(n, L)), dtype=torch.uint8, device=dev)
            self.info = torch.empty(L, dtype=torch.int32, device=dev)
        args = (spec, _lib.ptr(self.x64), self.x64.shape[1], n, L, _lib.ptr(self.p), _lib.ptr(self.nz),
                _lib.ptr(self.info), _lib.ptr(self.ws), _lib.ctypes.c_void_p(stream.cuda_stream))
        self._fut = None
        if _ASYNC_FACTOR and not torch.cuda.is_current_stream_capturing():
            dix = dev.index if dev.index is not None else torch.cuda.current_device()

            def enqueue():
                torch.cuda.set_device(dix)
                return lib.lvae_kl_closed_factor_f32(*args)
            self._fut = _factor_pool().submit(enqueue)
        else:
            _lib.check(lib.lvae_kl_closed_factor_f32(*args), "kl_closed_factor")
        self.stream = stream
        self.n, self.L = n, L
        self.consumed = False

    def wait_enqueued(self):
        if self._fut is not None:
            rc = self._fut.result()
            self._fut = None
            _lib.check(rc, "kl_closed_factor")

    def join(self):
        self.wait_enqueued()
        cur = torch.cuda.current_stream(self.ws.device)
        cur.wait_stream(self.stream)
        for t in (self.ws, self.info, self.x64, self.p, self.nz):
            t.record_stream(cur)


def kl_closed_prefactor(covar_modules, train_x, likelihoods, L, stream):
    spec, params = _stack_modules(covar_modules)
    if params.shape[0] != L:
        raise ValueError(f"kernel batch {params.shape[0]} != latent dims {L}")
    noise = _noise_vector(likelihoods, L).to(params.device)
    return KLFactor(spec, params, noise, train_x, stream)


class _KLState:
    ws = p = x64 = spec = None
    n = L = 0


_refine_log = None


@contextlib.contextmanager
def kl_closed_refine_log():
    global _refine_log
    prev, _refine_log = _refine_log, []
    try:
        yield _refine_log
    finally:
        _refine_log = prev


_hyper_log = None


@contextlib.contextmanager
def kl_closed_hyper_log():
    global _hyper_log
    prev, _hyper_log = _hyper_log, []
    try:
        yield _hyper_log
    finally:
        _hyper_log = prev


def _log_refine(lib, ws, n, L, dev):
    est = torch.zeros(L, dtype=torch.float64, device=dev)
    flag = torch.zeros(L, dtype=torch.int32, device=dev)
    _lib.check(lib.lvae_kl_closed_refine_state(n, L, _lib.ptr(ws), _lib.ptr(est), _lib.ptr(flag), _lib.stream_ptr()),
               "kl_closed_refine_state")
    _refine_log.append((est, flag))


class _KLHyperFn(torch.autograd.Function):

    @staticmethod
    def forward(ctx, params, noise, state, L):
        ctx.state = state
        ctx.in_dtypes = (params.dtype, noise.dtype, noise.shape)
        return torch.zeros(L, dtype=torch.float64, device=params.device)

    @staticmethod
    def backward(ctx, gkl):
        lib = _lib.lib()
        st = ctx.state
        if st.ws is None:
            raise RuntimeError("KL_closed: the hyper-parameter backward ran twice (its workspace is released "
                               "after the first; use retain_graph only for the (mu, logvar) half)")
        g = gkl.detach().to(torch.float64).reshape(st.L).contiguous()
        dp = torch.empty_like(st.p)
        dnz = torch.empty(st.L, dtype=torch.float64, device=st.p.device)
        rc = lib.lvae_kl_closed_bwd_hyper_f32(st.spec, _lib.ptr(st.x64), st.x64.shape[1], st.n, st.L, _lib.ptr(st.p),
                                              _lib.ptr(g), _lib.ptr(dp), _lib.ptr(dnz), _lib.ptr(st.ws),
                                              _lib.stream_ptr())
        _lib.check(rc, "kl_closed_bwd_hyper")
        st.ws = st.p = st.x64 = None
        pd, nd, nshape = ctx.in_dtypes
        return dp.to(pd), dnz.to(nd).reshape(nshape), None, None


class _KLClosedFn(torch.autograd.Function):

    @staticmethod
    def forward(ctx, params, noise, mu, logv, x, spec, factor, state, need_bwd):
        lib = _lib.lib()
        n, L = mu.shape
        dev = mu.device
        mu64 = mu.detach().to(torch.float64).contiguous()
        lv64 = logv.detach().to(torch.float64).contiguous()
        kl = torch.empty(L, dtype=torch.float64, device=dev)
        if factor is not None:
            if factor.n != n or factor.L != L:
                raise ValueError(f"factor is for n={factor.n}, L={factor.L}; got n={n}, L={L}")
            factor.join()
            x64, p, ws, info = factor.x64, factor.p, factor.ws, factor.info
            rc = lib.lvae_kl_closed_reduce_f32(spec, _lib.ptr(x64), x64.shape[1], n, L, _lib.ptr(p), _lib.ptr(factor.nz),
                                               _lib.ptr(mu64), _lib.ptr(lv64), L, _lib.ptr(kl), _lib.ptr(ws),
                                               need_bwd, _lib.stream_ptr())
            _lib.check(rc, "kl_closed_reduce")
        else:
            x64 = x.detach().to(torch.float64).contiguous()
            p = params.detach().to(torch.float64).contiguous()
            nz = noise.detach().to(torch.float64).reshape(L).contiguous()
            ws = torch.empty(int(lib.lvae_kl_closed_workspace_size(n, L)), dtype=torch.uint8, device=dev)
            info = torch.empty(L, dtype=torch.int32, device=dev)
            rc = lib.lvae_kl_closed_fwd_f32(spec, _lib.ptr(x64), x64.shape[1], n, L, _lib.ptr(p), _lib.ptr(nz),
                                            _lib.ptr(mu64), _lib.ptr(lv64), L, _lib.ptr(kl), _lib.ptr(info),
                                            _lib.ptr(ws), need_bwd, _lib.stream_ptr())
            _lib.check(rc, "kl_closed_fwd")
        _check_info(info, "KL_closed cholesky")
        if _refine_log is not None:
            _log_refine(lib, ws, n, L, dev)
        if _hyper_log is not None:
            on = torch.zeros(1, dtype=torch.int32, device=dev)
            _lib.check(lib.lvae_kl_closed_hyper_state(n, L, _lib.ptr(ws), _lib.ptr(on), _lib.stream_ptr()),
                       "kl_closed_hyper_state")
            _hyper_log.append(on)
        state.ws, state.p, state.x64, state.spec, state.n, state.L = ws, p, x64, spec, n, L
        ctx.save_for_backward(lv64, ws)
        ctx.in_dtypes = (mu.dtype, logv.dtype)
        return kl

    @staticmethod
    def backward(ctx, gkl):
        lib = _lib.lib()
        lv64, ws = ctx.saved_tensors
        n, L = lv64.shape
        g = gkl.detach().to(torch.float64).reshape(L).contiguous()
        dmu = torch.empty_like(lv64)
        dlv = torch.empty_like(lv64)
        rc = lib.lvae_kl_closed_bwd_latent_f32(n, L, _lib.ptr(lv64), L, _lib.ptr(g), _lib.ptr(dmu), _lib.ptr(dlv),
                                               _lib.ptr(ws), _lib.stream_ptr())
        _lib.check(rc, "kl_closed_bwd_latent")
        md, ld = ctx.in_dtypes
        return None, None, dmu.to(md), dlv.to(ld), None, None, None, None, None


def _kl_closed_apply(params, noise, mu, log_var, train_x, spec, factor):
    L = mu.shape[1]
    need_bwd = int(torch.is_grad_enabled() and any(t.requires_grad for t in (params, noise, mu, log_var)))
    state = _KLState()
    hyper = None
    if torch.is_grad_enabled() and (params.requires_grad or noise.requires_grad):
        hyper = _KLHyperFn.apply(params, noise, state, L)
    kl = _KLClosedFn.apply(params.detach(), noise.detach(), mu, log_var, train_x, spec, factor, state, need_bwd)
    return kl if hyper is None else kl + hyper


def _stack_modules(covar_modules):
    if isinstance(covar_modules, (list, tuple, torch.nn.ModuleList)):
        specs, ps = zip(*[kernel_spec_and_params(k) for k in covar_modules])
        return specs[0], torch.cat(ps, 0)
    return kernel_spec_and_params(covar_modules)


def _noise_vector(likelihoods, L):
    if isinstance(likelihoods, (list, tuple, torch.nn.ModuleList)):
        return torch.cat([lk.noise.reshape(-1) for lk in likelihoods]).reshape(L)
    nz = likelihoods.noise.reshape(-1)
    return nz.expand(L) if nz.numel() == 1 else nz


def KL_closed_batched(covar_modules, train_x, likelihoods, mu, log_var, factor=None):
    L = mu.shape[1]
    if factor is not None:
        if factor.consumed:
            raise RuntimeError("KL_closed_batched: this KLFactor was already used (one reduce per factor: "
                               "launch a new kl_closed_prefactor for each step)")
        factor.consumed = True
        return _kl_closed_apply(factor.params, factor.noise, mu, log_var, train_x, factor.spec, factor)
    spec, params = _stack_modules(covar_modules)
    if params.shape[0] != L:
        raise ValueError(f"kernel batch {params.shape[0]} != latent dims {L}")
    noise = _noise_vector(likelihoods, L).to(params.device)
    return _kl_closed_apply(params, noise, mu, log_var, train_x, spec, None)


def KL_closed(covar_module, train_x, likelihoods, data, mu, log_var):
    n = data.shape[0]
    return KL_closed_batched(covar_module, train_x[:n], likelihoods, mu.reshape(n, 1), log_var.reshape(n, 1))[0]


class _HensmanPre:

    def __init__(self, params0, params1, noise, m, H, x, z, spec0, spec1, dims, want_ng, dev):
        lib = _lib.lib()
        f64 = lambda t: t.detach().to(torch.float64).contiguous()
        self.p0, self.p1, self.nz = f64(params0), f64(params1), f64(noise).reshape(-1)
        self.m64, self.H64, self.x64, self.z64 = f64(m), f64(H), f64(x), f64(z)
        L, M = dims.L, dims.M
        self.ws = torch.empty(int(lib.lvae_hensman_workspace_size(dims)), dtype=torch.uint8, device=dev)
        self.kld = torch.empty((), dtype=torch.float64, device=dev)
        self.gm = torch.empty(L, M, 1, dtype=torch.float64, device=dev) if want_ng else None
        self.gH = torch.empty(L, M, M, dtype=torch.float64, device=dev) if want_ng else None
        self.info = torch.empty(L, dtype=torch.int32, device=dev)
        self.spec0, self.spec1, self.dims = spec0, spec1, dims

    def run(self, part, mu64=None, lv64=None):
        rc = _lib.lib().lvae_hensman_fwd_part_f64(
            part, self.spec0, self.spec1, self.dims, _lib.ptr(self.x64), _lib.ptr(self.z64), _lib.ptr(self.m64),
            _lib.ptr(self.H64), _lib.ptr(mu64), _lib.ptr(lv64), _lib.ptr(self.p0), _lib.ptr(self.p1),
            _lib.ptr(self.nz), _lib.ptr(self.kld), _lib.ptr(self.gm), _lib.ptr(self.gH), _lib.ptr(self.info),
            _lib.ptr(self.ws), _lib.stream_ptr())
        _lib.check(rc, "hensman_fwd")


class HensmanPrior:

    def __init__(self, covar_module0, covar_module1, likelihood, latent_dim, m, H, train_xt, z, P_tot, P_batch, T,
                 natural_gradient, eps, ng_prior_share=1.0, stream=None):
        a = _hensman_args(covar_module0, covar_module1, likelihood, latent_dim, H, train_xt, z, P_tot, P_batch, T,
                          natural_gradient, eps, ng_prior_share)
        self.params0, self.params1, self.noise, self.zz, self.spec0, self.spec1, self.dims = a
        self.m, self.H, self.x = m, H, train_xt
        self.want_ng = bool(natural_gradient)
        self.stream = stream
        if stream is not None:
            stream.wait_stream(torch.cuda.current_stream(train_xt.device))
        with torch.cuda.stream(stream) if stream is not None else contextlib.nullcontext():
            self.pre = _HensmanPre(self.params0, self.params1, self.noise, m, H, train_xt, self.zz, self.spec0,
                                   self.spec1, self.dims, self.want_ng, train_xt.device)
            self.pre.run(1)
        self.consumed = False

    def join(self):
        if self.stream is None:
            return
        cur = torch.cuda.current_stream(self.pre.ws.device)
        cur.wait_stream(self.stream)
        pre = self.pre
        for t in (pre.p0, pre.p1, pre.nz, pre.m64, pre.H64, pre.x64, pre.z64, pre.ws, pre.kld, pre.gm, pre.gH,
                  pre.info):
            if t is not None:
                t.record_stream(cur)


class _HensmanFn(torch.autograd.Function):
    @staticmethod
    def forward(ctx, params0, params1, noise, mu, logv, m, H, x, z, spec0, spec1, dims, want_ng, pre=None):
        dev = mu.device
        f64 = lambda t: t.detach().to(torch.float64).contiguous()
        mu64, lv64 = f64(mu), f64(logv)
        L, M = dims.L, dims.M
        if pre is None:
            pre = _HensmanPre(params0, params1, noise, m, H, x, z, spec0, spec1, dims, want_ng, dev)
            pre.run(0, mu64, lv64)
        else:
            pre.run(2, mu64, lv64)
        lib = _lib.lib()
        p0, p1, nz, m64, H64, x64, z64, ws = pre.p0, pre.p1, pre.nz, pre.m64, pre.H64, pre.x64, pre.z64, pre.ws
        kld, gm, gH, info = pre.kld, pre.gm, pre.gH, pre.info
        _check_info(info, "minibatch_KLD_upper_bound cholesky (10000+col: K0zz, 20000+col: B_st, 30000+col: H)")
        ctx.save_for_backward(p0, p1, nz, mu64, lv64, m64, H64, x64, z64, ws)
        ctx.spec0, ctx.spec1, ctx.dims = spec0, spec1, dims
        ctx.dtypes = (params0.dtype, params1.dtype, noise.dtype, noise.shape, mu.dtype, logv.dtype, m.dtype, H.dtype)
        ctx.z_dtype = z.dtype
        if want_ng:
            off = int(lib.lvae_hensman_iH_offset(dims))
            gH._lvae_iH = (ws[off:off + L * M * M * 8].view(torch.float64).view(L, M, M), H, H._version)
            ctx.mark_non_differentiable(gm, gH)
            return kld, gm, gH
        return kld, None, None

    @staticmethod
    def backward(ctx, gkld, _gm=None, _gH=None):
        lib = _lib.lib()
        p0, p1, nz, mu64, lv64, m64, H64, x64, z64, ws = ctx.saved_tensors
        d = ctx.dims
        g = gkld.detach().to(torch.float64).reshape(1).contiguous()
        dmu, dlv = torch.empty_like(mu64), torch.empty_like(lv64)
        dp0, dp1 = torch.empty_like(p0), torch.empty_like(p1)
        dnz = torch.empty_like(nz)
        adam = not d.natural_gradient
        dm = torch.empty_like(m64) if adam else None
        dH = torch.empty_like(H64) if adam else None
        rc = lib.lvae_hensman_bwd_f64(ctx.spec0, ctx.spec1, d, _lib.ptr(x64), _lib.ptr(z64), _lib.ptr(m64),
                                      _lib.ptr(H64), _lib.ptr(mu64), _lib.ptr(lv64), _lib.ptr(p0), _lib.ptr(p1),
                                      _lib.ptr(nz), _lib.ptr(g), _lib.ptr(dmu), _lib.ptr(dlv), _lib.ptr(dp0),
                                      _lib.ptr(dp1), _lib.ptr(dnz), _lib.ptr(dm), _lib.ptr(dH), _lib.ptr(ws),
                                      _lib.stream_ptr())
        _lib.check(rc, "hensman_bwd")
        t0, t1, tn, nshape, tmu, tlv, tm, tH = ctx.dtypes
        dz = None
        if ctx.needs_input_grad[8]:
            from .gpapprox import _bound_dz
            dz = _bound_dz("hensman", lib.lvae_hensman_bwd_z_f64, ctx.spec0, d, x64, z64, p0, ws, d.P_b * d.T,
                           ctx.z_dtype)
        return (dp0.to(t0), dp1.to(t1), dnz.to(tn).reshape(nshape), dmu.to(tmu), dlv.to(tlv),
                None if dm is None else dm.to(tm), None if dH is None else dH.to(tH),
                None, dz, None, None, None, None, None)


def minibatch_KLD_upper_bound(covar_module0, covar_module1, likelihood, latent_dim, m, H, train_xt, mu, log_v, z,
                              P_tot, P_batch, T, natural_gradient, eps, ng_prior_share=1.0, prior=None):
    if prior is not None:
        if prior.consumed:
            raise RuntimeError("minibatch_KLD_upper_bound: this HensmanPrior was already used")
        prior.consumed = True
        prior.join()
        return _HensmanFn.apply(prior.params0, prior.params1, prior.noise, mu, log_v, prior.m, prior.H, prior.x,
                                prior.zz, prior.spec0, prior.spec1, prior.dims, prior.want_ng, prior.pre)
    a = _hensman_args(covar_module0, covar_module1, likelihood, latent_dim, H, train_xt, z, P_tot, P_batch, T,
                      natural_gradient, eps, ng_prior_share)
    params0, params1, noise, zz, spec0, spec1, dims = a
    return _HensmanFn.apply(params0, params1, noise, mu, log_v, m, H, train_xt, zz, spec0, spec1, dims,
                            bool(natural_gradient))


def _hensman_args(covar_module0, covar_module1, likelihood, latent_dim, H, train_xt, z, P_tot, P_batch, T,
                  natural_gradient, eps, ng_prior_share):
    spec0, params0 = kernel_spec_and_params(covar_module0)
    spec1, params1 = kernel_spec_and_params(covar_module1)
    L, M = latent_dim, H.shape[-1]
    if params0.shape[0] == 1 and L > 1:
        params0 = params0.expand(L, -1)
    if params1.shape[0] == 1 and L > 1:
        params1 = params1.expand(L, -1)
    noise = likelihood.noise_covar.noise.reshape(-1)
    if noise.numel() == 1 and L > 1:
        noise = noise.expand(L)
    Q = train_xt.shape[-1]
    if train_xt.shape[0] != P_batch * T:
        raise ValueError(f"train_xt has {train_xt.shape[0]} rows, expected P_batch*T = {P_batch * T}")
    zz = z if z.dim() == 3 else z.unsqueeze(0).expand(L, -1, -1)
    dims = _lib.HensmanDims(L, M, int(P_batch), int(T), int(Q), float(P_tot), float(eps), int(bool(natural_gradient)),
                            float(ng_prior_share))
    return params0, params1, noise, zz, spec0, spec1, dims


def _subject_layout(ids):
    ids_c = ids.detach().to("cpu", torch.float64)
    subjects = torch.unique(ids_c)
    rows = [torch.nonzero(ids_c == s_, as_tuple=False).reshape(-1) for s_ in subjects]
    T_max = max(int(r.numel()) for r in rows)
    gather = torch.empty(len(rows), T_max, dtype=torch.int64)
    valid = torch.zeros(len(rows), T_max, dtype=torch.bool)
    for p, r in enumerate(rows):
        gather[p, :r.numel()] = r
        gather[p, r.numel():] = r[0]
        valid[p, :r.numel()] = True
    seg = torch.tensor([int(r.numel()) for r in rows], dtype=torch.int32)
    return gather.reshape(-1), valid.reshape(-1), seg, T_max


def minibatch_KLD_upper_bound_iter(covar_module0, covar_module1, likelihood, latent_dim, m, H, train_xt, mu, log_v,
                                   z, P, P_in_current_batch, N, natural_gradient, id_covariate, eps,
                                   ng_prior_share=1.0):
    spec0, params0 = kernel_spec_and_params(covar_module0)
    spec1, params1 = kernel_spec_and_params(covar_module1)
    L, M = latent_dim, H.shape[-1]
    if params0.shape[0] == 1 and L > 1:
        params0 = params0.expand(L, -1)
    if params1.shape[0] == 1 and L > 1:
        params1 = params1.expand(L, -1)
    noise = likelihood.noise_covar.noise.reshape(-1)
    if noise.numel() == 1 and L > 1:
        noise = noise.expand(L)
    dev = mu.device
    gather, valid, seg, T_max = _subject_layout(train_xt[:, id_covariate])
    P_b = int(seg.numel())
    gather_d = gather.to(dev)
    keep = valid.to(dev, mu.dtype).unsqueeze(1)
    x_pad = train_xt.detach()[gather_d]
    mu_pad = mu[gather_d] * keep
    lv_pad = log_v[gather_d] * keep.to(log_v.dtype)
    seg_d = seg.to(dev)
    zz = z if z.dim() == 3 else z.unsqueeze(0).expand(L, -1, -1)
    p_tot = float(P) * P_b / float(P_in_current_batch)
    dims = _lib.HensmanDims(L, M, P_b, int(T_max), int(train_xt.shape[-1]), p_tot, float(eps),
                            int(bool(natural_gradient)), float(ng_prior_share), seg_d.data_ptr(), float(N))
    dims.keepalive = seg_d
    kld, gm, gH = _HensmanFn.apply(params0, params1, noise, mu_pad, lv_pad, m, H, x_pad, zz, spec0, spec1, dims,
                                   bool(natural_gradient))
    return kld, gm, gH


def natural_gradient_update_(m, H, grad_m, grad_H, natural_gradient_lr):
    if not (m.dtype == H.dtype == torch.float64 and m.is_contiguous() and H.is_contiguous() and m.is_cuda):
        return False
    lib = _lib.lib()
    L, M = H.shape[0], H.shape[-1]
    gm = grad_m.detach().to(torch.float64).contiguous()
    gH = grad_H.detach().to(torch.float64).contiguous()
    ws = torch.empty(int(lib.lvae_natgrad_workspace_size(L, M)), dtype=torch.uint8, device=H.device)
    info = torch.empty(L, dtype=torch.int32, device=H.device)
    iH = None
    cached = getattr(grad_H, "_lvae_iH", None)
    if cached is not None and cached[1] is H and cached[1]._version == cached[2]:
        iH = cached[0]
    with torch.no_grad():
        rc = lib.lvae_natgrad_update_f64(L, M, _lib.ptr(m.detach()), _lib.ptr(H.detach()), _lib.ptr(gm), _lib.ptr(gH),
                                         float(natural_gradient_lr), _lib.ptr(iH), _lib.ptr(info), _lib.ptr(ws),
                                         _lib.stream_ptr())
    _lib.check(rc, "natgrad_update")
    from torch.autograd.graph import increment_version
    increment_version(m)
    increment_version(H)
    _check_info(info, "natural-gradient update cholesky")
    return True


def natural_gradient_update(m, H, grad_m, grad_H, natural_gradient_lr):
    lib = _lib.lib()
    L, M = H.shape[0], H.shape[-1]
    m2 = m.detach().to(torch.float64).contiguous().clone()
    H2 = H.detach().to(torch.float64).contiguous().clone()
    gm = grad_m.detach().to(torch.float64).contiguous()
    gH = grad_H.detach().to(torch.float64).contiguous()
    ws = torch.empty(int(lib.lvae_natgrad_workspace_size(L, M)), dtype=torch.uint8, device=H.device)
    info = torch.empty(L, dtype=torch.int32, device=H.device)
    iH = None
    cached = getattr(grad_H, "_lvae_iH", None)
    if cached is not None and cached[1] is H and cached[1]._version == cached[2]:
        iH = cached[0]
    rc = lib.lvae_natgrad_update_f64(L, M, _lib.ptr(m2), _lib.ptr(H2), _lib.ptr(gm), _lib.ptr(gH),
                                     float(natural_gradient_lr), _lib.ptr(iH), _lib.ptr(info), _lib.ptr(ws),
                                     _lib.stream_ptr())
    _lib.check(rc, "natgrad_update")
    _check_info(info, "natural-gradient update cholesky")
    return m2.reshape(m.shape), H2
```

### longitudinal-vae_amd/lvae_amd/steps.py

```python
import contextlib
import os
import weakref

import torch

from .elbo import (KL_closed_batched, kl_closed_prefactor, minibatch_KLD_upper_bound, natural_gradient_update,
                   natural_gradient_update_, take_pending)


_BWD_ON_CALLER = os.environ.get("LVAE_BWD_ON_CALLER", "1") != "0"


def bwd_thread_ctx():
    return torch.autograd.set_multithreading_enabled(False) if _BWD_ON_CALLER else contextlib.nullcontext()


def _graph_vae_default():
    import os
    return os.environ.get("LVAE_GRAPH_VAE", "0") == "1"


class ClosedStep:
    def __init__(self, vae, kernel, likelihood, optimiser, weight=0.15, loss_function="mse",
                 constrain_scales=True, grad_hook=None, vae_stream_priority=-1, graph_vae=None):
        self.vae, self.kernel, self.lik, self.opt = vae, kernel, likelihood, optimiser
        from .vae import GraphedConvVAE
        self.gvae = GraphedConvVAE(vae) if (_graph_vae_default() if graph_vae is None else graph_vae) else None
        self.weight, self.loss_function, self.constrain_scales = weight, loss_function, constrain_scales
        self.grad_hook = grad_hook
        self.vae_stream_priority = vae_stream_priority

    def _stream(self, name, device):
        s = getattr(self, name, None)
        if s is None or s.device != device:
            s = torch.cuda.Stream(device=device, priority=self.vae_stream_priority)
            setattr(self, name, s)
            from .vae import lend_early_stream
            lend_early_stream(device)
        return s

    def forward_backward(self, img, mask, X, eps=None):
        with bwd_thread_ctx():
            return self._forward_backward(img, mask, X, eps)

    def _forward_backward(self, img, mask, X, eps=None):
        self.opt.zero_grad(set_to_none=True)
        if img.is_cuda:
            main = torch.cuda.current_stream(img.device)
            capturing = torch.cuda.is_current_stream_capturing()
            vst = self._stream("_vae_stream", img.device)
            vst.wait_stream(main)
            factor = kl_closed_prefactor(self.kernel, X, self.lik, self.vae.latent_dim, main)
            enc_done = torch.cuda.Event()
            mse_mode = self.loss_function == "mse"
            with torch.cuda.stream(vst):
                gv = None if capturing else self.gvae
                if gv is not None:
                    mu, log_var = gv.encode(img, mask)
                else:
                    mu, log_var = self.vae.encode(img)
                enc_done.record(vst)
                z = self.vae.sample_latent(mu, log_var, eps)
                zd = z.detach().requires_grad_()
                if gv is not None:
                    recon_loss, nll_loss = gv.decode_loss(zd, img, mask)
                else:
                    recon = self.vae.decode(zd)
                    mse, nll = self.vae.loss_function(recon, img, mask)
                    recon_loss, nll_loss = mse.sum(), nll.sum()
                rec_term = recon_loss if mse_mode else nll_loss
                rec_term.backward()
            factor.wait_enqueued()
            main.wait_event(enc_done)
            mu.record_stream(main)
            log_var.record_stream(main)
            kl = KL_closed_batched(self.kernel, X, self.lik, mu, log_var, factor=factor)
            L = mu.shape[1]
            if mse_mode:
                gp = kl.sum() / L
                gp_term = self.weight * gp
            else:
                gp = kl.sum()
                gp_term = gp
            with torch.cuda.stream(vst):
                torch.autograd.backward([z, gp_term], [zd.grad, None])
            main.wait_stream(vst)
            for t in (recon_loss, nll_loss, rec_term):
                t.record_stream(main)
            net = rec_term.detach() + gp_term.detach()
            return net, recon_loss.detach().clone(), nll_loss.detach().clone(), gp.detach()
        else:
            recon, mu, log_var = self.vae(img, eps)
            mse, nll = self.vae.loss_function(recon, img, mask)
            recon_loss, nll_loss = mse.sum(), nll.sum()
            kl = KL_closed_batched(self.kernel, X, self.lik, mu, log_var)
        L = mu.shape[1]
        if self.loss_function == "mse":
            gp = kl.sum() / L
            net = recon_loss + self.weight * gp
        else:
            gp = kl.sum()
            net = nll_loss + gp
        net.backward()
        return net.detach(), recon_loss.detach(), nll_loss.detach(), gp.detach()

    def communicate(self):
        if self.grad_hook is not None:
            self.grad_hook()

    def apply(self):
        self.opt.step()
        if self.constrain_scales:
            self.lik.noise = 1.0

    def __call__(self, img, mask, X, eps=None):
        out = self.forward_backward(img, mask, X, eps)
        self.communicate()
        self.apply()
        return out


class _StepTermsFn(torch.autograd.Function):

    @staticmethod
    def forward(ctx, mse, nll, kld, c, ks, w, use_nll):
        from . import _lib
        lib = _lib.lib()
        dev = mse.device
        m, n, k = mse.contiguous(), nll.contiguous(), kld.detach().to(torch.float64).contiguous()
        rec, nl = torch.empty((), device=dev), torch.empty((), device=dev)
        net, kd = torch.empty((), dtype=torch.float64, device=dev), torch.empty((), dtype=torch.float64, device=dev)
        _lib.check(lib.lvae_step_terms_fwd(_lib.ptr(m), _lib.ptr(n), m.numel(), _lib.ptr(k), float(c), float(ks),
                                           float(w), int(use_nll), _lib.ptr(rec), _lib.ptr(nl), _lib.ptr(net),
                                           _lib.ptr(kd), _lib.stream_ptr()), "step_terms_fwd")
        ctx.set_materialize_grads(False)
        ctx.meta = (float(c), float(ks), float(w), int(use_nll), m.numel(), kld.shape, kld.dtype)
        return net, rec, nl, kd

    @staticmethod
    def backward(ctx, g_net, g_rec, g_nl, g_kd):
        from . import _lib
        lib = _lib.lib()
        c, ks, w, use_nll, B, kshape, kdtype = ctx.meta
        dev = next(g for g in (g_net, g_rec, g_nl, g_kd) if g is not None).device
        f64 = lambda g: None if g is None else g.detach().to(torch.float64).contiguous()
        f32 = lambda g: None if g is None else g.detach().to(torch.float32).contiguous()
        gn, gr, gl, gk = f64(g_net), f32(g_rec), f32(g_nl), f64(g_kd)
        g_mse, g_nll = torch.empty((), device=dev), torch.empty((), device=dev)
        g_kld = torch.empty((), dtype=torch.float64, device=dev)
        _lib.check(lib.lvae_step_terms_bwd(_lib.ptr(gn), _lib.ptr(gr), _lib.ptr(gl), _lib.ptr(gk), c, ks, w, use_nll,
                                           _lib.ptr(g_mse), _lib.ptr(g_nll), _lib.ptr(g_kld), _lib.stream_ptr()),
                   "step_terms_bwd")
        return (g_mse.expand(B), g_nll.expand(B), g_kld.reshape(kshape).to(kdtype), None, None, None, None)


class HensmanStep:

    def __init__(self, vae, k0, k1, likelihood, optimiser, m, H, z, P_tot, T, weight=0.15, loss_function="mse",
                 natural_gradient=True, natural_gradient_lr=0.01, eps=1e-6, world=1, grad_hook=None,
                 ng_reduce=None):
        self.vae, self.k0, self.k1, self.lik, self.opt = vae, k0, k1, likelihood, optimiser
        if z.requires_grad:
            import warnings
            warnings.warn("HensmanStep keeps the inducing inputs fixed: z.requires_grad is ignored here (z.grad stays "
                          "None); DuboStep / ElboStep or an eager loop over minibatch_KLD_upper_bound train z",
                          stacklevel=2)
        self.m, self.H, self.z = m, H, z.detach()
        self.P_tot, self.T = P_tot, T
        self.weight, self.loss_function = weight, loss_function
        self.ng, self.ng_lr, self.eps = natural_gradient, natural_gradient_lr, eps
        self.world, self.grad_hook, self.ng_reduce = world, grad_hook, ng_reduce
        self._gm = self._gH = None

    def forward_backward(self, img, mask, X, eps=None):
        self.opt.zero_grad(set_to_none=True)
        recon, mu, log_var = self.vae(img, eps)
        mse, nll = self.vae.loss_function(recon, img, mask)
        L = mu.shape[1]
        P_b = X.shape[0] // self.T
        PSD_H = self.H if self.ng else self.H @ self.H.transpose(-1, -2)
        kld, gm, gH = minibatch_KLD_upper_bound(self.k0, self.k1, self.lik, L, self.m, PSD_H, X, mu, log_var,
                                                self.z, self.P_tot, P_b, self.T, self.ng, self.eps,
                                                ng_prior_share=1.0 / self.world)
        mse_loss = self.loss_function == "mse"
        if mse.is_cuda and mse.dtype == nll.dtype == torch.float32 and kld.numel() == 1:
            net, recon_loss, nll_loss, kld = _StepTermsFn.apply(mse, nll, kld, self.P_tot / P_b,
                                                                1.0 / L if mse_loss else 1.0, self.weight,
                                                                not mse_loss)
        else:
            recon_loss = mse.sum() * self.P_tot / P_b
            nll_loss = nll.sum() * self.P_tot / P_b
            if mse_loss:
                kld = kld / L
                net = recon_loss + self.weight * kld
            else:
                net = nll_loss + kld
        net.backward()
        self._gm, self._gH = gm, gH
        return net.detach(), recon_loss.detach(), nll_loss.detach(), kld.detach()

    def communicate(self):
        if self.grad_hook is not None:
            self.grad_hook()
        if self.ng and self.ng_reduce is not None:
            self.ng_reduce([self._gm, self._gH])

    def apply(self):
        self.opt.step()
        if self.ng:
            if not natural_gradient_update_(self.m, self.H, self._gm, self._gH, self.ng_lr):
                m2, H2 = natural_gradient_update(self.m, self.H, self._gm, self._gH, self.ng_lr)
                with torch.no_grad():
                    self.m.copy_(m2.reshape(self.m.shape).to(self.m.dtype))
                    self.H.copy_(H2.to(self.H.dtype))

    def __call__(self, img, mask, X, eps=None):
        out = self.forward_backward(img, mask, X, eps)
        self.communicate()
        self.apply()
        return out


class _VaryingLayout:

    def __init__(self, T, id_covariate, who):
        if T is None and id_covariate is None:
            raise ValueError(f"{who}: T=None (subjects of varying length) needs id_covariate")
        self.id_covariate = id_covariate
        self.builds = 0
        self._key, self._layout = None, None

    def __call__(self, X):
        from .gpapprox import subject_layout
        if self._key is None or self._key[0]() is not X or self._key[1] != X._version:
            self._layout = subject_layout(X[:, self.id_covariate])
            self._key = (weakref.ref(X), X._version)
            self.builds += 1
        return self._layout


class DuboStep:

    def __init__(self, vae, k0, k1, likelihood, optimiser, z, T, weight=0.15, loss_function="mse", eps=1e-6,
                 constrain_scales=True, grad_hook=None, id_covariate=None):
        self.vae, self.k0, self.k1, self.lik, self.opt = vae, k0, k1, likelihood, optimiser
        self.z, self.T = z, T
        self.layout = _VaryingLayout(T, id_covariate, "DuboStep") if T is None else None
        self.weight, self.loss_function, self.eps = weight, loss_function, eps
        self.constrain_scales, self.grad_hook = constrain_scales, grad_hook

    def forward_backward(self, img, mask, X, eps=None):
        from .gpapprox import deviance_upper_bound_batched, deviance_upper_bound_varying_T
        self.opt.zero_grad(set_to_none=True)
        recon, mu, log_var = self.vae(img, eps)
        mse, nll = self.vae.loss_function(recon, img, mask)
        recon_loss, nll_loss = mse.sum(), nll.sum()
        L = mu.shape[1]
        if self.T is None:
            dubo = deviance_upper_bound_varying_T(L, self.k0, self.k1, self.lik, X, mu, log_var, self.z,
                                                  self.layout.id_covariate, self.eps, layout=self.layout(X))
        else:
            dubo = deviance_upper_bound_batched(L, self.k0, self.k1, self.lik, X, mu, log_var, self.z,
                                                X.shape[0] // self.T, self.T, self.eps)
        if self.loss_function == "mse":
            gp = dubo.sum() / L
            net = recon_loss + self.weight * gp
        else:
            gp = dubo.sum()
            net = nll_loss + gp
        net.backward()
        return net.detach(), recon_loss.detach(), nll_loss.detach(), gp.detach()

    def communicate(self):
        if self.grad_hook is not None:
            self.grad_hook()

    def apply(self):
        self.opt.step()
        if self.constrain_scales:
            for lk in (self.lik if isinstance(self.lik, (list, tuple, torch.nn.ModuleList)) else [self.lik]):
                lk.noise = 1.0

    def __call__(self, img, mask, X, eps=None):
        out = self.forward_backward(img, mask, X, eps)
        self.communicate()
        self.apply()
        return out


class ElboStep:

    def __init__(self, vae, k0, k1, likelihood, optimiser, z, T, weight=0.15, loss_function="mse", eps=1e-6,
                 constrain_scales=True, grad_hook=None, num_samples=1, id_covariate=None):
        self.vae, self.k0, self.k1, self.lik, self.opt = vae, k0, k1, likelihood, optimiser
        self.z, self.T = z, T
        self.layout = _VaryingLayout(T, id_covariate, "ElboStep") if T is None else None
        self.weight, self.loss_function, self.eps = weight, loss_function, eps
        self.constrain_scales, self.grad_hook = constrain_scales, grad_hook
        self.num_samples = int(num_samples)

    def forward_backward(self, img, mask, X, eps=None, eps_gp=None):
        from .gpapprox import elbo_batched, elbo_varying_T
        self.opt.zero_grad(set_to_none=True)
        recon, mu, log_var = self.vae(img, eps)
        mse, nll = self.vae.loss_function(recon, img, mask)
        recon_loss, nll_loss = mse.sum(), nll.sum()
        L, S = mu.shape[1], self.num_samples
        if eps_gp is None:
            eps_gp = torch.randn((S,) + tuple(mu.shape), dtype=mu.dtype, device=mu.device)
        if tuple(eps_gp.shape) != (S,) + tuple(mu.shape):
            raise ValueError(f"eps_gp must be [{S}, {mu.shape[0]}, {L}], got {tuple(eps_gp.shape)}")
        Z = torch.stack([self.vae.sample_latent(mu, log_var, eps_gp[s]) for s in range(S)])
        if self.T is None:
            el = elbo_varying_T(L, self.k0, self.k1, self.lik, X, Z, self.z, self.layout.id_covariate, self.eps,
                                layout=self.layout(X))
        else:
            el = elbo_batched(L, self.k0, self.k1, self.lik, X, Z, self.z, X.shape[0] // self.T, self.T, self.eps)
        if self.loss_function == "mse":
            gp = -el.sum() / (S * L)
            net = recon_loss + self.weight * gp
        else:
            gp = -el.sum() / S
            net = nll_loss + gp
        net.backward()
        return net.detach(), recon_loss.detach(), nll_loss.detach(), gp.detach()

    def communicate(self):
        if self.grad_hook is not None:
            self.grad_hook()

    def apply(self):
        self.opt.step()
        if self.constrain_scales:
            for lk in (self.lik if isinstance(self.lik, (list, tuple, torch.nn.ModuleList)) else [self.lik]):
                lk.noise = 1.0

    def __call__(self, img, mask, X, eps=None, eps_gp=None):
        out = self.forward_backward(img, mask, X, eps, eps_gp)
        self.communicate()
        self.apply()
        return out


def _comm_capturable():
    import os
    import torch.distributed as dist
    if os.environ.get("LVAE_GRAPH_COMM", "0") != "1":
        return False
    return dist.is_available() and dist.is_initialized() and dist.get_backend() == "nccl"


class GraphedStep:

    def __init__(self, step, inputs, warmup=3, shared_pool=False, capture_comm=None):
        self.step, self.inputs = step, inputs
        if getattr(step, "gvae", None) is not None:
            step.gvae = None
        comm = getattr(step, "grad_hook", None) is not None or getattr(step, "ng_reduce", None) is not None
        if capture_comm is None:
            capture_comm = _comm_capturable()
        if comm and capture_comm:
            comm = False
        self.stream = torch.cuda.Stream()
        self.stream.wait_stream(torch.cuda.current_stream())
        with torch.cuda.stream(self.stream):
            for _ in range(warmup):
                step(*inputs)
        torch.cuda.current_stream().wait_stream(self.stream)
        torch.cuda.synchronize()
        take_pending()
        self.g1 = torch.cuda.CUDAGraph()
        with torch.cuda.graph(self.g1, stream=self.stream):
            self.out = step.forward_backward(*inputs)
            if not comm:
                step.communicate()
                step.apply()
        self.g2 = None
        if comm:
            self.g2 = torch.cuda.CUDAGraph()
            with torch.cuda.graph(self.g2, stream=self.stream, pool=self.g1.pool() if shared_pool else None):
                step.apply()
        self.pending = take_pending()
        self.comm = comm

    def __call__(self):
        self.g1.replay()
        if self.comm:
            self.step.communicate()
# ... 7 lines not shown
```

Before: 123.2.

## Chain KL latent gradients into reduce and fork refine-diag onto side stream

Adds a KL chain path. The latent prep kernel now runs on the VAE stream right after encoding and also writes per-block sqrt-variance maxima, so the bscale kernel reads a short max vector instead of scanning all of sv. The reduce computes dmu and dlogv in-line using a precomputed gradient scale and records an event so the encoder backward can start before the KL finalize, instead of waiting for a separate autograd backward pass. The refine-diagonal work is forked onto a side stream to overlap with the gram residual and alpha kernels. This adds complexity through event and stream ordering and a separate refine partials buffer, and the path is disabled under graph capture or when the graphed VAE is used.

```diff
diff --git a/include/lvae_hip.h b/include/lvae_hip.h
--- a/include/lvae_hip.h
+++ b/include/lvae_hip.h
@@ -76,6 +76,13 @@
                               const double* params, const double* noise, const double* mu, const double* logv,
                               int ld_mu, double* kl, void* workspace, int need_bwd, void* stream);
 
+int lvae_kl_closed_prep_f32(int n, int L, const void* mu, const void* logv, int ld_mu, int is_f64, void* workspace,
+                            void* stream);
+int lvae_kl_closed_reduce_latent_f32(const lvae_kernel_spec* spec, const double* x, int ldx, int n, int L,
+                                     const double* params, const double* noise, const void* mu, const void* logv,
+                                     int ld_mu, int is_f64, int prepped, double* kl, const double* g, void* dmu,
+                                     void* dlogv, void* workspace, int need_bwd, void* latent_event, void* stream);
+
 int lvae_kl_closed_bwd_f32(const lvae_kernel_spec* spec, const double* x, int ldx, int n, int L,
                            const double* params, const double* mu, const double* logv, int ld_mu,
                            const double* gkl, double* dmu, double* dlogv, double* dparams, double* dnoise,
@@ -92,6 +99,9 @@
 
 int lvae_kl_closed_resid_state(int n, int L, const void* workspace, int32_t* covflag, int32_t* binned,
                                void* stream);
+
+int lvae_kl_closed_latent_state(int n, int L, const void* workspace, double* mu, float* v, float* sv, float* bsc,
+                                double* alpha, double* kdiag, void* stream);
 
 size_t lvae_spd_inv_chol_scratch_size(int np_, int L);
 int lvae_spd_inv_chol_f32(int np_, int L, float* A, void* scratch, float* Ainv, double* logdet, int32_t* info,
diff --git a/longitudinal-vae_amd/csrc/chol_inv.hip b/longitudinal-vae_amd/csrc/chol_inv.hip
--- a/longitudinal-vae_amd/csrc/chol_inv.hip
+++ b/longitudinal-vae_amd/csrc/chol_inv.hip
@@ -1723,7 +1723,7 @@
   return 0;
 }
 
-__global__ __launch_bounds__(64) void ci_bscale_kernel(CiScratch S, const float* __restrict__ sv, int np_,
+__global__ __launch_bounds__(64) void ci_bscale_kernel(CiScratch S, const float* __restrict__ svmax, int np_,
                                                        float* __restrict__ bsc) {
   const int l = blockIdx.x, t = threadIdx.x, nt = S.nt;
   const float* ys = S.ysc + (int64_t)l * nt * nt;
@@ -1737,7 +1737,7 @@
     d = fmaxf(d, c);
   }
   float v = 0.f;
-  for (int i = t; i < np_; i += 64) v = fmaxf(v, sv[(int64_t)l * np_ + i]);
+  for (int b = t; b < nt; b += 64) v = fmaxf(v, svmax[(int64_t)l * nt + b]);
 #pragma unroll
   for (int o = 32; o > 0; o >>= 1) {
     d = fmaxf(d, __shfl_xor(d, o, 64));
@@ -1747,7 +1747,7 @@
 }
 
 int ci_lauum_f32(int np_, int L, void* scratch, const _Float16* YT, float* Kinv, const double* mu, const float* sv,
-                 float* apart, _Float16* Bh, float* bsc, hipStream_t st, const int* hbon) {
+                 float* apart, _Float16* Bh, float* bsc, hipStream_t st, const int* hbon, const float* svmax) {
   if (np_ <= 0 || np_ % kSwB || np_ / kSwB > 64) return -1;
   CiScratch S((char*)scratch, np_, L);
   const int nt = S.nt, per = nt * (nt + 1) / 2, nwg = per * L;
@@ -1763,7 +1763,7 @@
     gl.bl_out = Bh ? Bh + full : nullptr;
     gl.bsc = bsc;
     gl.hbon = hbon;
-    if (Bh) ci_bscale_kernel<<<L, 64, 0, st>>>(S, sv, np_, bsc);
+    if (Bh) ci_bscale_kernel<<<L, 64, 0, st>>>(S, svmax, np_, bsc);
     ci_gemm_kernel<kCiLauumKL><<<nwg, 512, 0, st>>>(gl, S);
   } else {
     ci_gemm_kernel<kCiLauum><<<nwg, 512, 0, st>>>(gl, S);
@@ -1795,7 +1795,7 @@
 int ci_inverse_f32(int np_, int L, float* A, void* scratch, _Float16* YT, float* Kinv, double* logdet,
                    int32_t* info, hipStream_t st) {
   LVAE_TRY(ci_factor_f32(np_, L, A, scratch, YT, Kinv, logdet, info, st));
-  return ci_lauum_f32(np_, L, scratch, YT, Kinv, nullptr, nullptr, nullptr, nullptr, nullptr, st, nullptr);
+  return ci_lauum_f32(np_, L, scratch, YT, Kinv, nullptr, nullptr, nullptr, nullptr, nullptr, st, nullptr, nullptr);
 }
 
 }
diff --git a/longitudinal-vae_amd/csrc/kl_closed.hip b/longitudinal-vae_amd/csrc/kl_closed.hip
--- a/longitudinal-vae_amd/csrc/kl_closed.hip
+++ b/longitudinal-vae_amd/csrc/kl_closed.hip
@@ -30,7 +30,7 @@
 int ci_factor_f32(int np_, int L, float* A, void* scratch, _Float16* YT, float* Kinv, double* logdet,
                   int32_t* info, hipStream_t st, float* lout = nullptr);
 int ci_lauum_f32(int np_, int L, void* scratch, const _Float16* YT, float* Kinv, const double* mu, const float* sv,
-                 float* apart, _Float16* Bh, float* bsc, hipStream_t st, const int* hbon);
+                 float* apart, _Float16* Bh, float* bsc, hipStream_t st, const int* hbon, const float* svmax);
 size_t ci_scratch_bytes(int np_, int L);
 size_t kl_resid_partials_bytes(int np_, int L);
 int kl_gram_resid(const lvae_kernel_spec* spec, const double* x, int ldx, int n, int np_, int L,
@@ -74,6 +74,8 @@
   double* ypart;
   double* yvec;
   double* K64e;
+  float* svmax;
+  double* fpart;
   size_t bytes, bytes_base;
   KLWorkspace(char* base, int np_, int L) {
     size_t off = 0;
@@ -108,6 +110,8 @@
     hbon = base ? reinterpret_cast<const int*>(kl_hyper_dev(hb, np_, L)) : nullptr;
     rest = (double*)take((size_t)L * sizeof(double));
     rflag = (int*)take((size_t)L * sizeof(int));
+    fpart = (double*)take(kl_refine_part_bytes(np_, L));
+    svmax = (float*)take((size_t)L * (np_ / 256) * sizeof(float));
     bytes_base = off;
     ypart = (double*)take(2 * (size_t)L * (np_ / 256) * np_ * sizeof(double));
     yvec = (double*)take((size_t)L * np_ * sizeof(double));
@@ -116,15 +120,33 @@
   }
 };
 
-__global__ void kl_prep_kernel(const double* __restrict__ mu, const double* __restrict__ logv, int ld, int n, int np_,
-                               int L, double* __restrict__ muc, float* __restrict__ v, float* __restrict__ sv) {
-  const int i = blockIdx.x * blockDim.x + threadIdx.x, l = blockIdx.y;
-  if (i >= np_) return;
+__device__ inline double lat_load(const void* p, int f64, int64_t e) {
+  return f64 ? static_cast<const double*>(p)[e] : (double)static_cast<const float*>(p)[e];
+}
+__device__ inline void lat_store(void* p, int f64, int64_t e, double val) {
+  if (f64) static_cast<double*>(p)[e] = val;
+  else static_cast<float*>(p)[e] = (float)val;
+}
+__device__ inline double kl_dlogv(double g, double lv, double kd) { return 0.5 * g * (exp(lv) * kd - 1.0); }
+
+__global__ __launch_bounds__(256) void kl_prep_kernel(const void* __restrict__ mu, const void* __restrict__ logv,
+                                                      int f64, int ld, int n, int np_, int L,
+                                                      double* __restrict__ muc, float* __restrict__ v,
+                                                      float* __restrict__ sv, float* __restrict__ svmax) {
+  __shared__ float wmax[4];
+  const int i = blockIdx.x * 256 + threadIdx.x, l = blockIdx.y;
   const bool in = i < n;
-  muc[(int64_t)l * np_ + i] = in ? mu[(int64_t)i * ld + l] : 0.0;
-  const double vv = in ? exp(logv[(int64_t)i * ld + l]) : 0.0;
+  muc[(int64_t)l * np_ + i] = in ? lat_load(mu, f64, (int64_t)i * ld + l) : 0.0;
+  const double vv = in ? exp(lat_load(logv, f64, (int64_t)i * ld + l)) : 0.0;
   v[(int64_t)l * np_ + i] = (float)vv;
-  sv[(int64_t)l * np_ + i] = (float)sqrt(vv);
+  float m = (float)sqrt(vv);
+  sv[(int64_t)l * np_ + i] = m;
+#pragma unroll
+  for (int o = 32; o > 0; o >>= 1) m = fmaxf(m, __shfl_xor(m, o, 64));
+  if ((threadIdx.x & 63) == 0) wmax[threadIdx.x >> 6] = m;
+  __syncthreads();
+  if (threadIdx.x == 0)
+    svmax[(int64_t)l * gridDim.x + blockIdx.x] = fmaxf(fmaxf(wmax[0], wmax[1]), fmaxf(wmax[2], wmax[3]));
 }
 
 __global__ __launch_bounds__(256) void kl_alpha0_kernel(const float* __restrict__ apart, const float* __restrict__ Kinv,
@@ -221,8 +243,11 @@
   }
 }
 
-__global__ __launch_bounds__(256) void kl_alpha_reduce(const double* __restrict__ part, const double* base, int np_,
-                                                       double* alpha) {
+__global__ __launch_bounds__(256) void kl_alpha_tail_kernel(const double* __restrict__ part, const double* base,
+                                                            int np_, double* alpha, const double* __restrict__ kdiag,
+                                                            const void* __restrict__ logv, int f64, int ld, int n,
+                                                            const double* __restrict__ g, void* __restrict__ dmu,
+                                                            void* __restrict__ dlogv) {
   const int i = blockIdx.x * 256 + threadIdx.x, l = blockIdx.y, nt = np_ / 64;
   if (i >= np_) return;
   double acc = 0.0;
@@ -236,7 +261,14 @@
     acc += v3;
   }
   const int64_t o = (int64_t)l * np_ + i;
-  alpha[o] = base[o] + acc;
+  const double a = base[o] + acc;
+  alpha[o] = a;
+  if (g && i < n) {
+    const int64_t e = (int64_t)i * ld + l;
+    const double gl = g[l];
+    lat_store(dmu, f64, e, gl * a);
+    lat_store(dlogv, f64, e, kl_dlogv(gl, lat_load(logv, f64, e), kdiag[o]));
+  }
 }
 
 template <bool UPPER, bool SUMSQ>
@@ -294,8 +326,8 @@
   out[o] = (base ? base[o] : 0.0) + acc;
 }
 
-__global__ __launch_bounds__(256) void kl_finalize_kernel(const double* __restrict__ muc, const double* __restrict__ logv,
-                                                          int ld, const double* __restrict__ alpha,
+__global__ __launch_bounds__(256) void kl_finalize_kernel(const double* __restrict__ muc, const void* __restrict__ logv,
+                                                          int f64, int ld, const double* __restrict__ alpha,
                                                           const double* __restrict__ kdiag,
                                                           const double* __restrict__ logdet, int n, int np_,
                                                           double* __restrict__ kl) {
@@ -303,7 +335,7 @@
   const int l = blockIdx.x, tid = threadIdx.x;
   double quad = 0.0, tr = 0.0, slv = 0.0;
   for (int i = tid; i < n; i += 256) {
-    const double lv = logv[(int64_t)i * ld + l];
+    const double lv = lat_load(logv, f64, (int64_t)i * ld + l);
     quad += muc[(int64_t)l * np_ + i] * alpha[(int64_t)l * np_ + i];
     tr += exp(lv) * kdiag[(int64_t)l * np_ + i];
     slv += lv;
@@ -314,16 +346,17 @@
   if (tid == 0) kl[l] = 0.5 * (tr + quad - (double)n + logdet[l] - slv);
 }
 
-__global__ void kl_bwd_elem_kernel(const double* __restrict__ logv, int ld, int n, int np_, int L,
+__global__ void kl_bwd_elem_kernel(const void* __restrict__ logv, int f64, int ld, int n, int np_, int L,
                                    const double* __restrict__ alpha, const double* __restrict__ kdiag,
-                                   const double* __restrict__ gkl, double* __restrict__ dmu,
-                                   double* __restrict__ dlogv) {
+                                   const double* __restrict__ gkl, void* __restrict__ dmu,
+                                   void* __restrict__ dlogv) {
   const int64_t e = (int64_t)blockIdx.x * blockDim.x + threadIdx.x;
   if (e >= (int64_t)n * L) return;
   const int i = (int)(e / L), l = (int)(e % L);
   const double g = gkl[l];
-  dmu[(int64_t)i * ld + l] = g * alpha[(int64_t)l * np_ + i];
-  dlogv[(int64_t)i * ld + l] = 0.5 * g * (exp(logv[(int64_t)i * ld + l]) * kdiag[(int64_t)l * np_ + i] - 1.0);
+  lat_store(dmu, f64, (int64_t)i * ld + l, g * alpha[(int64_t)l * np_ + i]);
+  lat_store(dlogv, f64, (int64_t)i * ld + l,
+            kl_dlogv(g, lat_load(logv, f64, (int64_t)i * ld + l), kdiag[(int64_t)l * np_ + i]));
 }
 
 }
@@ -449,21 +482,41 @@
   }
 }
 
-int lvae_kl_closed_reduce_f32(const lvae_kernel_spec* spec, const double* x, int ldx, int n, int L,
-                              const double* params, const double* noise, const double* mu, const double* logv,
-                              int ld_mu, double* kl, void* workspace, int need_bwd, void* stream) {
-  LVAE_TRY(kl_check_problem(spec, x, ldx, n, L, params));
-  if (!noise) return -7;
-  if (!mu) return -8;
-  if (!logv) return -9;
-  if (ld_mu < L) return -10;
-  if (!kl) return -11;
-  if (kl_bad_ws(workspace)) return -12;
-  hipStream_t st = (hipStream_t)stream;
+static bool kl_chain_env() {
+  const char* e = getenv("LVAE_KL_CHAIN");
+  return !e || atoi(e) != 0;
+}
+
+static int kl_prep(const void* mu, const void* logv, int f64, int ld_mu, int n, int L, void* workspace,
+                   hipStream_t st) {
   const int np_ = lvae_kl_closed_padded_n(n);
   KLWorkspace ws((char*)workspace, np_, L);
+  kl_prep_kernel<<<dim3(np_ / 256, L), 256, 0, st>>>(mu, logv, f64, ld_mu, n, np_, L, ws.mu, ws.v, ws.sv, ws.svmax);
+  LVAE_CHECK_LAUNCH();
+  return 0;
+}
+
+int lvae_kl_closed_prep_f32(int n, int L, const void* mu, const void* logv, int ld_mu, int is_f64, void* workspace,
+                            void* stream) {
+  if (n <= 0 || n > kKlMaxN) return -1;
+  if (L <= 0) return -2;
+  if (!mu) return -3;
+  if (!logv) return -4;
+  if (ld_mu < L) return -5;
+  if (is_f64 != 0 && is_f64 != 1) return -6;
+  if (kl_bad_ws(workspace)) return -7;
+  return kl_prep(mu, logv, is_f64, ld_mu, n, L, workspace, (hipStream_t)stream);
+}
+
+static int kl_reduce(const lvae_kernel_spec* spec, const double* x, int ldx, int n, int L, const double* params,
+                     const double* noise, const void* mu, const void* logv, int ld_mu, int f64, int prepped, double* kl,
+                     const double* g, void* dmu, void* dlogv, void* workspace, int need_bwd, hipEvent_t latent_event,
+                     hipStream_t st) {
+  const int np_ = lvae_kl_closed_padded_n(n);
+  KLWorkspace ws((char*)workspace, np_, L);
+  auto ok = [](hipError_t e) { return e == hipSuccess; };
   ProfScope ps(LVAE_PH_KL_REDUCE, st);
-  kl_prep_kernel<<<dim3(cdiv(np_, 256), L), 256, 0, st>>>(mu, logv, ld_mu, n, np_, L, ws.mu, ws.v, ws.sv);
+  if (!prepped) LVAE_TRY(kl_prep(mu, logv, f64, ld_mu, n, L, workspace, st));
   const bool rb_on = kl_resid_bins_enabled(spec, n);
   if (kl_early(workspace)) {
     const float* ysc = ci_ysc_ptr(ws.chol, np_, L);
@@ -475,15 +528,36 @@
     kl_ymv(ws, ysc, np_, L, true, ws.yvec, ws.alpha, ws.alpha, nullptr, st);
     LVAE_TRY(kl_refine_gate(spec, x, ldx, n, np_, L, params, noise, ws.kdiag, ws.rest, ws.rflag, st));
     LVAE_TRY(ci_lauum_flagged_f32(np_, L, ws.chol, ws.planes, ws.Kinv, ws.rflag, st));
-    LVAE_TRY(kl_refine_apply(spec, x, ldx, n, np_, L, params, noise, ws.Kinv, ws.kdiag, ws.K64e, ws.rpart, ws.rflag,
+    LVAE_TRY(kl_refine_apply(spec, x, ldx, n, np_, L, params, noise, ws.Kinv, ws.kdiag, ws.K64e, ws.fpart, ws.rflag,
                              st));
-    kl_finalize_kernel<<<L, 256, 0, st>>>(ws.mu, logv, ld_mu, ws.alpha, ws.kdiag, ws.logdet, n, np_, kl);
+    if (g) {
+      const int64_t tot = (int64_t)n * L;
+      kl_bwd_elem_kernel<<<cdiv(tot, 256), 256, 0, st>>>(logv, f64, ld_mu, n, np_, L, ws.alpha, ws.kdiag, g, dmu,
+                                                         dlogv);
+      if (latent_event && !ok(hipEventRecord(latent_event, st))) return LVAE_ERR_LAUNCH;
+    }
+    kl_finalize_kernel<<<L, 256, 0, st>>>(ws.mu, logv, f64, ld_mu, ws.alpha, ws.kdiag, ws.logdet, n, np_, kl);
     LVAE_CHECK_LAUNCH();
     return 0;
   }
+  hipStreamCaptureStatus cap = hipStreamCaptureStatusNone;
+  if (!ok(hipStreamIsCapturing(st, &cap))) return LVAE_ERR_LAUNCH;
+  const bool fork = kl_chain_env() && cap == hipStreamCaptureStatusNone;
+  std::unique_lock<std::recursive_mutex> lock(side_mutex(), std::defer_lock);
+  SideStream* sd = nullptr;
+  if (fork) {
+    lock.lock();
+    LVAE_TRY(side_stream(sd));
+  }
   LVAE_TRY(ci_lauum_f32(np_, L, ws.chol, ws.planes, ws.Kinv, ws.mu, ws.sv, ws.apart, need_bwd ? ws.Bp : nullptr,
-                        ws.bsc, st, ws.hbon));
+                        ws.bsc, st, ws.hbon, ws.svmax));
   kl_alpha0_kernel<<<dim3(np_ / 256, L), 256, 0, st>>>(ws.apart, ws.Kinv, np_, ws.alpha, ws.kdiag);
+  if (fork) {
+    if (!ok(hipEventRecord(sd->rfork, st)) || !ok(hipStreamWaitEvent(sd->s, sd->rfork, 0))) return LVAE_ERR_LAUNCH;
+    LVAE_TRY(kl_refine_diag(spec, x, ldx, n, np_, L, params, noise, ws.Kinv, ws.kdiag, ws.K64, ws.fpart, ws.rest,
+                            ws.rflag, sd->s));
+    if (!ok(hipEventRecord(sd->rjoin, sd->s))) return LVAE_ERR_LAUNCH;
+  }
   LVAE_TRY(kl_gram_resid(spec, x, ldx, n, np_, L, params, noise, ws.alpha, ws.mu, ws.rpart, ws.res,
                          rb_on ? ws.rb : nullptr, st));
   {
@@ -491,13 +565,52 @@
     int G = (LVAE_ALPHA_WG + L - 1) / L;
     G = G < ntiles ? G : ntiles;
     kl_alpha_sym_kernel<<<dim3(G, L), 256, 0, st>>>(ws.Kinv, ws.res, np_, ws.rpart, ntiles);
-    kl_alpha_reduce<<<dim3(np_ / 256, L), 256, 0, st>>>(ws.rpart, ws.alpha, np_, ws.alpha);
-  }
-  LVAE_TRY(kl_refine_diag(spec, x, ldx, n, np_, L, params, noise, ws.Kinv, ws.kdiag, ws.K64, ws.rpart, ws.rest,
-                          ws.rflag, st));
-  kl_finalize_kernel<<<L, 256, 0, st>>>(ws.mu, logv, ld_mu, ws.alpha, ws.kdiag, ws.logdet, n, np_, kl);
+  }
+  if (fork) {
+    if (!ok(hipStreamWaitEvent(st, sd->rjoin, 0))) return LVAE_ERR_LAUNCH;
+  } else {
+    LVAE_TRY(kl_refine_diag(spec, x, ldx, n, np_, L, params, noise, ws.Kinv, ws.kdiag, ws.K64, ws.fpart, ws.rest,
+                            ws.rflag, st));
+  }
+  kl_alpha_tail_kernel<<<dim3(np_ / 256, L), 256, 0, st>>>(ws.rpart, ws.alpha, np_, ws.alpha, ws.kdiag, logv, f64,
+                                                           ld_mu, n, g, dmu, dlogv);
+  if (g && latent_event && !ok(hipEventRecord(latent_event, st))) return LVAE_ERR_LAUNCH;
+  kl_finalize_kernel<<<L, 256, 0, st>>>(ws.mu, logv, f64, ld_mu, ws.alpha, ws.kdiag, ws.logdet, n, np_, kl);
   LVAE_CHECK_LAUNCH();
   return 0;
+}
+
+int lvae_kl_closed_reduce_f32(const lvae_kernel_spec* spec, const double* x, int ldx, int n, int L,
+                              const double* params, const double* noise, const double* mu, const double* logv,
+                              int ld_mu, double* kl, void* workspace, int need_bwd, void* stream) {
+  LVAE_TRY(kl_check_problem(spec, x, ldx, n, L, params));
+  if (!noise) return -7;
+  if (!mu) return -8;
+  if (!logv) return -9;
+  if (ld_mu < L) return -10;
+  if (!kl) return -11;
+  if (kl_bad_ws(workspace)) return -12;
+  return kl_reduce(spec, x, ldx, n, L, params, noise, mu, logv, ld_mu, 1, 0, kl, nullptr, nullptr, nullptr, workspace,
+                   need_bwd, nullptr, (hipStream_t)stream);
+}
+
+int lvae_kl_closed_reduce_latent_f32(const lvae_kernel_spec* spec, const double* x, int ldx, int n, int L,
+                                     const double* params, const double* noise, const void* mu, const void* logv,
+                                     int ld_mu, int is_f64, int prepped, double* kl, const double* g, void* dmu,
+                                     void* dlogv, void* workspace, int need_bwd, void* latent_event, void* stream) {
+  LVAE_TRY(kl_check_problem(spec, x, ldx, n, L, params));
+  if (!noise) return -7;
+  if (!mu) return -8;
+  if (!logv) return -9;
+  if (ld_mu < L) return -10;
+  if (is_f64 != 0 && is_f64 != 1) return -11;
+  if (prepped != 0 && prepped != 1) return -12;
+  if (!kl) return -13;
+  if (g && !dmu) return -15;
+  if (g && !dlogv) return -16;
+  if (kl_bad_ws(workspace)) return -17;
+  return kl_reduce(spec, x, ldx, n, L, params, noise, mu, logv, ld_mu, is_f64, prepped, kl, g, dmu, dlogv, workspace,
+                   need_bwd, (hipEvent_t)latent_event, (hipStream_t)stream);
 }
 
 int lvae_kl_closed_fwd_f32(const lvae_kernel_spec* spec, const double* x, int ldx, int n, int L, const double* params,
@@ -528,7 +641,8 @@
   KLWorkspace ws((char*)workspace, np_, L);
   if (kl_early(workspace)) {
     ProfScope ps(LVAE_PH_KL_REDUCE, st);
-    LVAE_TRY(ci_lauum_f32(np_, L, ws.chol, ws.planes, ws.Kinv, ws.mu, ws.sv, ws.apart, ws.Bp, ws.bsc, st, ws.hbon));
+    LVAE_TRY(ci_lauum_f32(np_, L, ws.chol, ws.planes, ws.Kinv, ws.mu, ws.sv, ws.apart, ws.Bp, ws.bsc, st, ws.hbon,
+                          ws.svmax));
   }
   float* S = reinterpret_cast<float*>(ws.planes);
   {
@@ -559,7 +673,7 @@
   KLWorkspace ws((char*)workspace, np_, L);
   ProfScope ps(LVAE_PH_BWD_ELEM, st);
   const int64_t tot = (int64_t)n * L;
-  kl_bwd_elem_kernel<<<cdiv(tot, 256), 256, 0, st>>>(logv, ld_mu, n, np_, L, ws.alpha, ws.kdiag, gkl, dmu, dlogv);
+  kl_bwd_elem_kernel<<<cdiv(tot, 256), 256, 0, st>>>(logv, 1, ld_mu, n, np_, L, ws.alpha, ws.kdiag, gkl, dmu, dlogv);
   LVAE_CHECK_LAUNCH();
   return 0;
 }
@@ -611,6 +725,25 @@
   return 0;
 }
 
+int lvae_kl_closed_latent_state(int n, int L, const void* workspace, double* mu, float* v, float* sv, float* bsc,
+                                double* alpha, double* kdiag, void* stream) {
+  if (n <= 0 || n > kKlMaxN) return -1;
+  if (L <= 0) return -2;
+  if (kl_bad_ws(workspace)) return -3;
+  const int np_ = lvae_kl_closed_padded_n(n);
+  KLWorkspace ws((char*)workspace, np_, L);
+  hipStream_t st = (hipStream_t)stream;
+  const size_t vec = (size_t)L * np_;
+  if ((mu && copy_words_async(mu, ws.mu, vec * sizeof(double), st) != 0) ||
+      (v && copy_words_async(v, ws.v, vec * sizeof(float), st) != 0) ||
+      (sv && copy_words_async(sv, ws.sv, vec * sizeof(float), st) != 0) ||
+      (bsc && copy_words_async(bsc, ws.bsc, (size_t)L * sizeof(float), st) != 0) ||
+      (alpha && copy_words_async(alpha, ws.alpha, vec * sizeof(double), st) != 0) ||
+      (kdiag && copy_words_async(kdiag, ws.kdiag, vec * sizeof(double), st) != 0))
+    return LVAE_ERR_LAUNCH;
+  return 0;
+}
+
 const char* lvae_version(void) { return "lvae_hip 0.1.0 gfx950"; }
 
 }
diff --git a/longitudinal-vae_amd/csrc/side_stream.cpp b/longitudinal-vae_amd/csrc/side_stream.cpp
--- a/longitudinal-vae_amd/csrc/side_stream.cpp
+++ b/longitudinal-vae_amd/csrc/side_stream.cpp
@@ -25,7 +25,7 @@
     if (hipGetDeviceProperties(&prop, dev) != hipSuccess) return LVAE_ERR_LAUNCH;
     sd.cus = prop.multiProcessorCount;
     for (hipEvent_t* e : {&sd.fork, &sd.prep, &sd.c, &sd.u2p[0], &sd.u2p[1], &sd.piv[0], &sd.piv[1], &sd.rbx, &sd.rb,
-                          &sd.efork, &sd.edone})
+                          &sd.efork, &sd.edone, &sd.rfork, &sd.rjoin})
       if (!*e && hipEventCreateWithFlags(e, hipEventDisableTiming) != hipSuccess) return LVAE_ERR_LAUNCH;
     if (hipStreamCreateWithPriority(&sd.s, hipStreamNonBlocking, greatest) != hipSuccess) return LVAE_ERR_LAUNCH;
   }
diff --git a/longitudinal-vae_amd/csrc/side_stream.hpp b/longitudinal-vae_amd/csrc/side_stream.hpp
--- a/longitudinal-vae_amd/csrc/side_stream.hpp
+++ b/longitudinal-vae_amd/csrc/side_stream.hpp
@@ -11,6 +11,7 @@
   hipEvent_t rbx = nullptr, rb = nullptr;
   hipStream_t early = nullptr;
   hipEvent_t efork = nullptr, edone = nullptr;
+  hipEvent_t rfork = nullptr, rjoin = nullptr;
   int cus = 0;
 };
 
diff --git a/longitudinal-vae_amd/lvae_amd/_lib.py b/longitudinal-vae_amd/lvae_amd/_lib.py
--- a/longitudinal-vae_amd/lvae_amd/_lib.py
+++ b/longitudinal-vae_amd/lvae_amd/_lib.py
@@ -97,6 +97,9 @@
     "lvae_kl_closed_factor_f32": (_I32, [_SPEC, _VP, _I32, _I32, _I32, _VP, _VP, _VP, _VP, _VP]),
     "lvae_kl_closed_reduce_f32": (_I32, [_SPEC, _VP, _I32, _I32, _I32, _VP, _VP, _VP, _VP, _I32, _VP, _VP, _I32,
                                          _VP]),
+    "lvae_kl_closed_prep_f32": (_I32, [_I32, _I32, _VP, _VP, _I32, _I32, _VP, _VP]),
+    "lvae_kl_closed_reduce_latent_f32": (_I32, [_SPEC, _VP, _I32, _I32, _I32, _VP, _VP, _VP, _VP, _I32, _I32, _I32, _VP,
+                                                _VP, _VP, _VP, _VP, _I32, _VP, _VP]),
     "lvae_kl_closed_fwd_f32": (_I32, [_SPEC, _VP, _I32, _I32, _I32, _VP, _VP, _VP, _VP, _I32, _VP, _VP, _VP,
                                       _I32, _VP]),
     "lvae_kl_closed_bwd_f32": (_I32, [_SPEC, _VP, _I32, _I32, _I32, _VP, _VP, _VP, _I32, _VP, _VP, _VP, _VP,
@@ -106,6 +109,7 @@
     "lvae_kl_closed_refine_state": (_I32, [_I32, _I32, _VP, _VP, _VP, _VP]),
     "lvae_kl_closed_hyper_state": (_I32, [_I32, _I32, _VP, _VP, _VP]),
     "lvae_kl_closed_resid_state": (_I32, [_I32, _I32, _VP, _VP, _VP, _VP]),
+    "lvae_kl_closed_latent_state": (_I32, [_I32, _I32, _VP, _VP, _VP, _VP, _VP, _VP, _VP, _VP]),
     "lvae_vae_loss_fwd_f32": (_I32, [_VP, _VP, _VP, _VP, _I32, _I32, _VP, _VP, _VP, _VP]),
     "lvae_vae_loss_bwd_partials": (_SZ, [_I32]),
     "lvae_bias_relu_fwd_f32": (_I32, [_VP, _VP, _I32, _I32, _I32, _VP]),
diff --git a/longitudinal-vae_amd/lvae_amd/elbo.py b/longitudinal-vae_amd/lvae_amd/elbo.py
--- a/longitudinal-vae_amd/lvae_amd/elbo.py
+++ b/longitudinal-vae_amd/lvae_amd/elbo.py
@@ -1,4 +1,5 @@
 import contextlib
+import ctypes
 import os
 
 import torch
@@ -83,6 +84,16 @@
         self.stream = stream
         self.n, self.L = n, L
         self.consumed = False
+        self.prepped = None
+
+    def prep(self, mu, log_var):
+        m, lv, f64 = _latent_views(mu, log_var)
+        if m.shape != (self.n, self.L):
+            raise ValueError(f"factor is for n={self.n}, L={self.L}; got {tuple(m.shape)}")
+        rc = _lib.lib().lvae_kl_closed_prep_f32(self.n, self.L, _lib.ptr(m), _lib.ptr(lv), m.stride(0), f64,
+                                                _lib.ptr(self.ws), _lib.stream_ptr())
+        _lib.check(rc, "kl_closed_prep")
+        self.prepped = (mu, log_var, m, lv, f64)
 
     def wait_enqueued(self):
         if self._fut is not None:
@@ -104,6 +115,72 @@
         raise ValueError(f"kernel batch {params.shape[0]} != latent dims {L}")
     noise = _noise_vector(likelihoods, L).to(params.device)
     return KLFactor(spec, params, noise, train_x, stream)
+
+
+def _latent_views(mu, log_var):
+    m, lv = mu.detach(), log_var.detach()
+    if m.dtype != lv.dtype or m.dtype not in (torch.float32, torch.float64):
+        m, lv = m.to(torch.float64), lv.to(torch.float64)
+    L = m.shape[1]
+    if not (m.stride(1) == lv.stride(1) == 1 and m.stride(0) == lv.stride(0) >= L):
+        m, lv = m.contiguous(), lv.contiguous()
+    return m, lv, int(m.dtype == torch.float64)
+
+
+class KLLatent:
+
+    def __init__(self, kl, dmu, dlogv, event, hyper):
+        self.kl, self.dmu, self.dlogv, self.event, self.hyper = kl, dmu, dlogv, event, hyper
+
+
+def _kl_closed_latent(factor, mu, log_var, g):
+    lib = _lib.lib()
+    n, L = mu.shape
+    dev = mu.device
+    if factor.n != n or factor.L != L:
+        raise ValueError(f"factor is for n={factor.n}, L={factor.L}; got n={n}, L={L}")
+    pre = factor.prepped
+    if pre is not None and pre[0] is mu and pre[1] is log_var:
+        m, lv, f64 = pre[2:]
+    else:
+        pre = None
+        m, lv, f64 = _latent_views(mu, log_var)
+    ld = m.stride(0)
+    factor.join()
+    cur = torch.cuda.current_stream(dev)
+    for t in (m, lv):
+        t.record_stream(cur)
+    g = g.detach().to(device=dev, dtype=torch.float64).reshape(L).contiguous()
+    kl = torch.empty(L, dtype=torch.float64, device=dev)
+    dmu = torch.empty((n, ld), dtype=m.dtype, device=dev)[:, :L]
+    dlv = torch.empty((n, ld), dtype=m.dtype, device=dev)[:, :L]
+    event = torch.cuda.Event()
+    event.record(cur)
+    params, noise = factor.params, factor.noise
+    state = _KLState()
+    hyper = None
+    if torch.is_grad_enabled() and (params.requires_grad or noise.requires_grad):
+        hyper = _KLHyperFn.apply(params, noise, state, L, False)
+    x64, p, ws = factor.x64, factor.p, factor.ws
+    rc = lib.lvae_kl_closed_reduce_latent_f32(factor.spec, _lib.ptr(x64), x64.shape[1], n, L, _lib.ptr(p),
+                                              _lib.ptr(factor.nz), _lib.ptr(m), _lib.ptr(lv), ld, f64,
+                                              int(pre is not None), _lib.ptr(kl), _lib.ptr(g), _lib.ptr(dmu),
+                                              _lib.ptr(dlv), _lib.ptr(ws), 1, ctypes.c_void_p(event.cuda_event),
+                                              _lib.stream_ptr())
+    _lib.check(rc, "kl_closed_reduce_latent")
+    _check_info(factor.info, "KL_closed cholesky")
+    if _refine_log is not None:
+        _log_refine(lib, ws, n, L, dev)
+    if _hyper_log is not None:
+        on = torch.zeros(1, dtype=torch.int32, device=dev)
+        _lib.check(lib.lvae_kl_closed_hyper_state(n, L, _lib.ptr(ws), _lib.ptr(on), _lib.stream_ptr()),
+                   "kl_closed_hyper_state")
+        _hyper_log.append(on)
+    state.ws, state.p, state.x64, state.spec, state.n, state.L = ws, p, x64, factor.spec, n, L
+    if m.dtype != mu.dtype:
+        dmu, dlv = dmu.to(mu.dtype), dlv.to(mu.dtype)
+        event.record(cur)
+    return KLLatent(kl, dmu, dlv, event, hyper)
 
 
 class _KLState:
@@ -148,9 +225,11 @@
 class _KLHyperFn(torch.autograd.Function):
 
     @staticmethod
-    def forward(ctx, params, noise, state, L):
+    def forward(ctx, params, noise, state, L, value=True):
         ctx.state = state
         ctx.in_dtypes = (params.dtype, noise.dtype, noise.shape)
+        if not value:
+            return torch.empty(L, dtype=torch.float64, device=params.device)
         return torch.zeros(L, dtype=torch.float64, device=params.device)
 
     @staticmethod
@@ -169,7 +248,7 @@
         _lib.check(rc, "kl_closed_bwd_hyper")
         st.ws = st.p = st.x64 = None
         pd, nd, nshape = ctx.in_dtypes
-        return dp.to(pd), dnz.to(nd).reshape(nshape), None, None
+        return dp.to(pd), dnz.to(nd).reshape(nshape), None, None, None
 
 
 class _KLClosedFn(torch.autograd.Function):
@@ -254,13 +333,17 @@
     return nz.expand(L) if nz.numel() == 1 else nz
 
 
-def KL_closed_batched(covar_modules, train_x, likelihoods, mu, log_var, factor=None):
+def KL_closed_batched(covar_modules, train_x, likelihoods, mu, log_var, factor=None, latent_scale=None):
     L = mu.shape[1]
+    if latent_scale is not None and factor is None:
+        raise ValueError("KL_closed_batched: latent_scale needs a launched factor (kl_closed_prefactor)")
     if factor is not None:
         if factor.consumed:
             raise RuntimeError("KL_closed_batched: this KLFactor was already used (one reduce per factor: "
                                "launch a new kl_closed_prefactor for each step)")
         factor.consumed = True
+        if latent_scale is not None:
+            return _kl_closed_latent(factor, mu, log_var, latent_scale)
         return _kl_closed_apply(factor.params, factor.noise, mu, log_var, train_x, factor.spec, factor)
     spec, params = _stack_modules(covar_modules)
     if params.shape[0] != L:
diff --git a/longitudinal-vae_amd/lvae_amd/steps.py b/longitudinal-vae_amd/lvae_amd/steps.py
--- a/longitudinal-vae_amd/lvae_amd/steps.py
+++ b/longitudinal-vae_amd/lvae_amd/steps.py
@@ -38,6 +38,13 @@
             from .vae import lend_early_stream
             lend_early_stream(device)
         return s
+
+    def _latent_scale(self, L, device):
+        key = (L, device, self.weight, self.loss_function)
+        if getattr(self, "_g_key", None) != key:
+            val = self.weight * (1.0 / L) if self.loss_function == "mse" else 1.0
+            self._g, self._g_key = torch.full((L,), val, dtype=torch.float64, device=device), key
+        return self._g
 
     def forward_backward(self, img, mask, X, eps=None):
         with bwd_thread_ctx():
@@ -53,12 +60,15 @@
             factor = kl_closed_prefactor(self.kernel, X, self.lik, self.vae.latent_dim, main)
             enc_done = torch.cuda.Event()
             mse_mode = self.loss_function == "mse"
+            gv = None if capturing else self.gvae
+            chain = not capturing and gv is None and os.environ.get("LVAE_KL_CHAIN", "1") != "0"
             with torch.cuda.stream(vst):
-                gv = None if capturing else self.gvae
                 if gv is not None:
                     mu, log_var = gv.encode(img, mask)
                 else:
                     mu, log_var = self.vae.encode(img)
+                if chain:
+                    factor.prep(mu, log_var)
                 enc_done.record(vst)
                 z = self.vae.sample_latent(mu, log_var, eps)
                 zd = z.detach().requires_grad_()
@@ -74,8 +84,13 @@
             main.wait_event(enc_done)
             mu.record_stream(main)
             log_var.record_stream(main)
-            kl = KL_closed_batched(self.kernel, X, self.lik, mu, log_var, factor=factor)
             L = mu.shape[1]
+            if chain:
+                g = self._latent_scale(L, img.device)
+                lat = KL_closed_batched(self.kernel, X, self.lik, mu, log_var, factor=factor, latent_scale=g)
+                kl = lat.kl
+            else:
+                kl = KL_closed_batched(self.kernel, X, self.lik, mu, log_var, factor=factor)
             if mse_mode:
                 gp = kl.sum() / L
                 gp_term = self.weight * gp
@@ -83,7 +98,20 @@
                 gp = kl.sum()
                 gp_term = gp
             with torch.cuda.stream(vst):
-                torch.autograd.backward([z, gp_term], [zd.grad, None])
+                if chain:
+                    vst.wait_event(lat.event)
+                    roots, grads = [z], [zd.grad]
+                    for t, d in ((mu, lat.dmu), (log_var, lat.dlogv)):
+                        if t.requires_grad:
+                            d.record_stream(vst)
+                            roots.append(t)
+                            grads.append(d)
+                    if lat.hyper is not None:
+                        roots.append(lat.hyper)
+                        grads.append(g)
+                    torch.autograd.backward(roots, grads)
+                else:
+                    torch.autograd.backward([z, gp_term], [zd.grad, None])
             main.wait_stream(vst)
             for t in (recon_loss, nll_loss, rec_term):
                 t.record_stream(main)
```

Measured after the change: 125.0 (median of 6 runs). 1.01x the previous value.
